# CameronDiao/MolCLR

Hardware: AMD Instinct MI355X
Metric: contrastive pre-train molecules/sec at batch 512, 1/2/4/8 MI355X; HBM GB/s on scatter_add (higher is better)
Workload: dtype f32; 1 GPU; c2: GIN 5x300 feat 512, batch 512/GPU, 10-50 atom graphs; model=gin 5x300 feat 512, global_batch=512, per_gpu_batch=512, mean_nodes_per_view=15278, mean_edges_per_view=25094, parallelism=dp1, views=one paired encoder pass, per-view BatchNorm statistics, augment=host: pre-built resident batch pairs

## Files before the change

### include/molclr.h

```cpp
#ifndef MOLCLR_H_
#define MOLCLR_H_

#include <stddef.h>
#include <stdint.h>

#ifdef __cplusplus
extern "C" {
#endif

typedef void* molclr_stream_t;

enum {
  MOLCLR_OK = 0,
  MOLCLR_ERR_ARG = -1,
  MOLCLR_ERR_WORKSPACE = -2,
  MOLCLR_ERR_UNSUPPORTED = -3
};

#define MOLCLR_NUM_ATOM_TYPE 119
#define MOLCLR_NUM_CHIRALITY 3
#define MOLCLR_NUM_BOND_TYPE 5
#define MOLCLR_NUM_BOND_DIR 3
#define MOLCLR_SELF_LOOP_BOND_TYPE 4
#define MOLCLR_ECOUNT_STRIDE 8
// ... 32 lines not shown
                             molclr_stream_t stream);

typedef struct molclr_stage_source {
  const int64_t *x, *edge_index, *edge_attr, *batch;
  int64_t num_nodes, num_edges;
} molclr_stage_source;
typedef struct molclr_graph_staged_segment {
  const int64_t* edge_index;
  const int64_t* edge_attr;
  const int64_t* batch;
  int64_t node_cap, edge_cap, num_graphs;
} molclr_graph_staged_segment;
int molclr_stage_segments(int nseg, const molclr_stage_source* src,
                          const molclr_graph_staged_segment* dst, int64_t* x_all,
                          int64_t num_nodes_cap, int64_t num_edges_cap, int64_t* counts,
                          molclr_stream_t stream);
int molclr_graph_build_dev(int nseg, const molclr_graph_staged_segment* segs, const int64_t* counts,
                           int64_t num_nodes_cap, int64_t num_edges_cap, int32_t* rowptr,
                           int32_t* col, uint8_t* ecode, int32_t* rowptr_t, int32_t* col_t,
                           uint32_t* nbr, uint32_t* nbr_t, int32_t* ecount, int32_t* graph_ptr,
                           int32_t* status, void* workspace, size_t workspace_bytes,
                           molclr_stream_t stream);

size_t molclr_mask_views_workspace_bytes(int64_t batch_size);
int molclr_mask_views(const int64_t* store_x, const int64_t* store_atom_ptr,
                      const int64_t* store_edge_index, const int64_t* store_edge_attr,
                      const int64_t* store_bond_ptr, int64_t store_mols, int64_t store_edges,
                      const int64_t* mol_ids, int64_t batch_size, uint64_t seed, int view,
                      int64_t* x_out, int64_t* edge_index_out, int64_t* edge_attr_out,
                      int64_t* batch_out, int64_t* ptr_out, int64_t num_nodes, int64_t num_edges,
                      int32_t* status, void* workspace, size_t workspace_bytes,
                      molclr_stream_t stream);

enum { MOLCLR_AUG_SUBGRAPH = 0, MOLCLR_AUG_MIX = 1 };
size_t molclr_aug_views_workspace_bytes(int64_t batch_size, int64_t num_nodes, int64_t num_bonds);
int molclr_aug_views_plan(const int64_t* store_atom_ptr, const int64_t* store_edge_index,
                          const int64_t* store_bond_ptr, int64_t store_mols, int64_t store_edges,
                          const int64_t* mol_ids, int64_t batch_size, uint64_t seed, int view,
                          int mode, int64_t num_nodes, int64_t num_bonds, int64_t* ptr_out,
                          int64_t* num_edges_out, int32_t* status, void* workspace,
                          size_t workspace_bytes, molclr_stream_t stream);
size_t molclr_aug_views_big_workspace_bytes(int64_t big_slots, int64_t big_atoms,
                                            int64_t big_bonds);
int molclr_aug_views_plan_big(const int64_t* store_atom_ptr, const int64_t* store_edge_index,
                              const int64_t* store_bond_ptr, int64_t store_mols,
                              int64_t store_edges, const int64_t* mol_ids, int64_t batch_size,
                              uint64_t seed, int view, int mode, int64_t num_nodes,
                              int64_t num_bonds, int64_t* ptr_out, int64_t* num_edges_out,
                              int32_t* status, void* workspace, size_t workspace_bytes,
                              int64_t big_slots, int64_t big_atoms, int64_t big_bonds,
                              void* big_workspace, size_t big_workspace_bytes,
                              molclr_stream_t stream);
int molclr_aug_views_write(const int64_t* store_x, const int64_t* store_atom_ptr,
                           const int64_t* store_edge_index, const int64_t* store_edge_attr,
                           const int64_t* store_bond_ptr, int64_t store_mols, int64_t store_edges,
                           const int64_t* mol_ids, int64_t batch_size, const int64_t* ptr,
                           int64_t num_nodes, int64_t num_bonds, int64_t num_edges, int64_t* x_out,
                           int64_t* edge_index_out, int64_t* edge_attr_out, int64_t* batch_out,
                           const void* workspace, size_t workspace_bytes, molclr_stream_t stream);

int molclr_atom_embed_fwd(const int64_t* x, const float* X1, const float* X2,
                          float* h, int64_t num_nodes, int64_t dim, int64_t n1,
                          int64_t n2, int32_t* status, molclr_stream_t stream);
size_t molclr_atom_embed_bwd_workspace_bytes(int64_t num_nodes, int64_t dim, int64_t n1,
                                             int64_t n2);
int molclr_atom_embed_bwd(const int64_t* x, const float* dh, float* dX1, float* dX2,
                          int64_t num_nodes, int64_t dim, int64_t n1, int64_t n2, int accumulate,
                          void* workspace, size_t workspace_bytes, molclr_stream_t stream);

#define MOLCLR_MAX_LAYERS 16
int molclr_edge_tables_combine(int layers, const float* const* E1s, const float* const* E2s,
                               float* Ec, int64_t dim, molclr_stream_t stream);

int molclr_gine_aggregate_fwd(const float* x, const int32_t* rowptr, const int32_t* col,
                              const uint8_t* ecode, const uint32_t* nbr, const float* Ec,
                              float* out, int64_t num_nodes, int64_t dim,
                              molclr_stream_t stream);
int64_t molclr_rowmax_layout(int64_t D);
size_t molclr_rowmax_bytes(int64_t N, int64_t D);
int molclr_gine_aggregate_fwd_rowmax(const float* x, const int32_t* rowptr, const int32_t* col,
                                     const uint8_t* ecode, const uint32_t* nbr, const float* Ec,
                                     float* out, int64_t N, int64_t D, float* rowparts,
                                     float* slot, molclr_stream_t stream);
size_t molclr_gine_aggregate_bwd_workspace_bytes(int64_t num_nodes, int64_t dim);
int molclr_gine_aggregate_bwd(const float* g, const int32_t* rowptr_t, const int32_t* col_t,
                              const uint32_t* nbr_t, const int32_t* ecount, float* dx, float* dE1, float* dE2,
                              int64_t num_nodes, int64_t dim, int accumulate, void* workspace,
                              size_t workspace_bytes, molclr_stream_t stream);

int molclr_gcn_aggregate_fwd(const float* xw, const int32_t* rowptr, const int32_t* col,
                             const uint8_t* ecode, const uint32_t* nbr, const float* E1,
                             const float* E2,
                             const float* bias, float* out, int64_t num_nodes,
                             int64_t dim, molclr_stream_t stream);
size_t molclr_gcn_aggregate_bwd_workspace_bytes(int64_t num_nodes, int64_t dim);
int molclr_gcn_aggregate_bwd(const float* g, const int32_t* rowptr_t, const int32_t* col_t,
                             const uint32_t* nbr_t, const int32_t* ecount, float* dxw, float* dE1, float* dE2,
                             float* dbias, int64_t num_nodes, int64_t dim, int accumulate,
                             void* workspace, size_t workspace_bytes, molclr_stream_t stream);

enum { MOLCLR_EPI_NONE = 0, MOLCLR_EPI_BIAS = 1, MOLCLR_EPI_BIAS_RELU = 2,
       MOLCLR_EPI_RELU_MASK = 3,
       MOLCLR_EPI_ACCUMULATE = 16  };
size_t molclr_gemm_f32_workspace_bytes(int64_t M, int64_t N, int64_t K);
int molclr_gemm_f32(const float* A, const float* B, float* C, int64_t M, int64_t N,
                    int64_t K, int64_t lda, int64_t ldb, int64_t ldc, int a_kmajor,
                    int b_kmajor, int epilogue_flags, const float* bias, const float* aux,
                    int64_t ldaux, void* workspace, size_t workspace_bytes,
                    molclr_stream_t stream);

int molclr_gemm_f32_impl(const float* A, const float* B, float* C, int64_t M, int64_t N,
                         int64_t K, int64_t lda, int64_t ldb, int64_t ldc, int a_kmajor,
                         int b_kmajor, int epilogue_flags, const float* bias, const float* aux,
                         int64_t ldaux, void* workspace, size_t workspace_bytes,
                         molclr_stream_t stream, int impl);

size_t molclr_bplanes_bytes(int64_t N, int64_t K);
int molclr_bplanes_make(const float* B, int64_t N, int64_t K, int64_t ldb, int b_kmajor,
                        uint16_t* planes, molclr_stream_t stream);
int molclr_bplanes_make_batch(int count, const float* const* B, const int64_t* N,
                              const int64_t* K, const int64_t* ldb, const int* b_kmajor,
                              uint16_t* const* planes, molclr_stream_t stream);
int molclr_gemm_f32_bplanes(const float* A, const uint16_t* planes, float* C, int64_t M,
                            int64_t N, int64_t K, int64_t lda, int64_t ldc, int a_kmajor,
                            int epilogue_flags, const float* bias, const float* aux,
                            int64_t ldaux, void* workspace, size_t workspace_bytes,
                            molclr_stream_t stream);
int molclr_gemm_f32_bplanes_tile(const float* A, const uint16_t* planes, float* C, int64_t M,
                                 int64_t N, int64_t K, int64_t lda, int64_t ldc, int a_kmajor,
                                 int epilogue_flags, const float* bias, const float* aux,
                                 int64_t ldaux, void* workspace, size_t workspace_bytes,
                                 molclr_stream_t stream, int tile);

size_t molclr_linear_wgrad_workspace_bytes(int64_t rows, int64_t n_out, int64_t n_in);
int molclr_linear_wgrad(const float* dy, const float* x, float* dW, float* db, int64_t rows,
                        int64_t n_out, int64_t n_in, int64_t ld_dy, int64_t ld_x, int accumulate,
                        void* workspace, size_t workspace_bytes, molclr_stream_t stream);
int molclr_linear_wgrad_groups(const float* dy, const float* x, float* dW, float* db,
                               int64_t rows, int64_t n_out, int64_t n_in, int64_t ld_dy,
                               int64_t ld_x, int accumulate, void* workspace,
                               size_t workspace_bytes, molclr_stream_t stream, int groups);

int molclr_absmax_f32(const float* x, int64_t rows, int64_t cols, int64_t ld, float* slot,
                      int accumulate, molclr_stream_t stream);
size_t molclr_hplanes_bytes(int64_t N, int64_t K);
int molclr_hplanes_make_batch(int count, const float* const* B, const int64_t* N,
                              const int64_t* K, const int64_t* ldb, const int* b_kmajor,
                              uint16_t* const* planes, molclr_stream_t stream);
int64_t molclr_gemm_row_parts(int64_t N);
int molclr_gemm_f32_bplanes_max(const float* A, const uint16_t* planes, float* C, int64_t M,
                                int64_t N, int64_t K, int64_t lda, int64_t ldc,
                                int epilogue_flags, const float* bias, const float* aux,
                                int64_t ldaux, float* amax_out, float* cmax, float* crow,
                                uint32_t* relu_bits, void* workspace, size_t workspace_bytes,
                                molclr_stream_t stream);
int molclr_absmax_rows_f32(const float* x, int64_t rows, int64_t cols, int64_t ld,
                           float* rowmax, float* slot, int accumulate, molclr_stream_t stream);
int molclr_gemm_f32_h3(const float* A, const float* amax, int a_row_parts, const uint16_t* hplanes,
                       float* C, int64_t M, int64_t N, int64_t K, int64_t lda, int64_t ldc,
                       int epilogue_flags, const float* bias, const float* aux, int64_t ldaux,
                       const uint32_t* mask_bits, float* cmax, float* crow, float* amax_out,
                       molclr_stream_t stream);
int molclr_gemm_f32_h3_impl(const float* A, const float* amax, int a_row_parts,
                            const uint16_t* hplanes, float* C, int64_t M, int64_t N, int64_t K,
                            int64_t lda, int64_t ldc, int epilogue_flags, const float* bias,
                            const float* aux, int64_t ldaux, const uint32_t* mask_bits, float* cmax,
                            float* crow, float* amax_out, uint32_t* relu_bits,
                            molclr_stream_t stream, int impl);
int molclr_gemm_f32_h3_bits(const float* A, const float* amax, int a_row_parts,
                            const uint16_t* hplanes, float* C, int64_t M, int64_t N, int64_t K,
                            int64_t lda, int64_t ldc, int epilogue_flags, const float* bias,
                            const float* aux, int64_t ldaux, const uint32_t* mask_bits,
                            float* cmax, float* crow, float* amax_out, uint32_t* relu_bits,
                            molclr_stream_t stream);
int molclr_linear_wgrad_h3_groups(const float* dy, const float* dymax, const float* x,
                                  const float* xmax, float* dW, float* db, int64_t rows,
                                  int64_t n_out, int64_t n_in, int64_t ld_dy, int64_t ld_x,
                                  int accumulate, void* workspace, size_t workspace_bytes,
                                  molclr_stream_t stream, int groups);
int molclr_linear_wgrad_h3(const float* dy, const float* dymax, const float* x,
                           const float* xmax, float* dW, float* db, int64_t rows, int64_t n_out,
                           int64_t n_in, int64_t ld_dy, int64_t ld_x, int accumulate,
                           void* workspace, size_t workspace_bytes, molclr_stream_t stream);
size_t molclr_linear_wgrad_h3_pair_workspace_bytes(int64_t rows, int64_t n_out_a, int64_t n_in_a,
                                                   int64_t n_out_b, int64_t n_in_b);
int molclr_linear_wgrad_h3_pair(const float* dy_a, const float* dymax_a, const float* x_a,
                                const float* xmax_a, float* dW_a, float* db_a, int64_t n_out_a,
                                int64_t n_in_a, int64_t ld_dy_a, int64_t ld_x_a,
                                const float* dy_b, const float* dymax_b, const float* x_b,
                                const float* xmax_b, float* dW_b, float* db_b, int64_t n_out_b,
                                int64_t n_in_b, int64_t ld_dy_b, int64_t ld_x_b, int64_t rows,
                                int accumulate, void* workspace, size_t workspace_bytes,
                                molclr_stream_t stream);

size_t molclr_colsum_f32_workspace_bytes(int64_t rows, int64_t cols);
int molclr_colsum_f32(const float* X, float* out, int64_t rows, int64_t cols, int64_t ld,
                      int accumulate, void* workspace, size_t workspace_bytes,
                      molclr_stream_t stream);

size_t molclr_batchnorm_workspace_bytes(int64_t rows, int64_t dim);
int molclr_batchnorm_fwd(const float* z, const float* gamma, const float* beta,
                         float* running_mean, float* running_var,
                         int64_t* num_batches_tracked, float* y,
                         float* save_mean, float* save_invstd, int64_t rows, int64_t dim,
                         double momentum, double eps, int training, int relu,
                         void* workspace, size_t workspace_bytes, molclr_stream_t stream);
int molclr_batchnorm_bwd(const float* dy, const float* z, const float* gamma,
                         const float* beta, const float* save_mean,
                         const float* save_invstd, float* dz, float* dgamma, float* dbeta,
                         int64_t rows, int64_t dim, int relu, int accumulate, void* workspace,
                         size_t workspace_bytes, molclr_stream_t stream);

enum { MOLCLR_DTYPE_F32 = 0, MOLCLR_DTYPE_BF16 = 1 };
size_t molclr_batchnorm_seg_workspace_bytes(int nseg, const int64_t* seg_rows, int64_t dim);
int molclr_batchnorm_seg_fwd(const void* z, const float* gamma, const float* beta,
                             float* running_mean, float* running_var,
                             int64_t* num_batches_tracked, void* y, float* save_mean,
                             float* save_invstd, int nseg, const int64_t* seg_rows, int64_t dim,
                             int dtype, double momentum, double eps, int training, int relu,
                             void* workspace, size_t workspace_bytes, molclr_stream_t stream);
int molclr_batchnorm_seg_bwd(const void* dy, const void* z, const float* gamma,
                             const float* beta, const float* save_mean, const float* save_invstd,
                             void* dz, float* dgamma, float* dbeta, int nseg,
                             const int64_t* seg_rows, int64_t dim, int dtype, int relu,
                             int accumulate, void* workspace, size_t workspace_bytes,
                             molclr_stream_t stream);

int molclr_bn_row_parts(int64_t dim);
size_t molclr_batchnorm_seg_dev_workspace_bytes(int nseg, int64_t rows_cap, int64_t dim);
int molclr_batchnorm_seg_fwd_dev(const void* z, const float* gamma, const float* beta,
                                 float* running_mean, float* running_var,
                                 int64_t* num_batches_tracked, void* y, float* save_mean,
                                 float* save_invstd, int nseg, const int64_t* seg_rows_dev,
                                 int64_t rows_cap, int64_t dim, int dtype, double momentum,
                                 double eps, int training, int relu, void* workspace,
                                 size_t workspace_bytes, molclr_stream_t stream);
int molclr_batchnorm_seg_bwd_dev(const void* dy, const void* z, const float* gamma,
                                 const float* beta, const float* save_mean,
                                 const float* save_invstd, void* dz, float* dgamma, float* dbeta,
                                 int nseg, const int64_t* seg_rows_dev, int64_t rows_cap,
                                 int64_t dim, int dtype, int relu, int accumulate, float* rowmax,
                                 float* slot, void* workspace, size_t workspace_bytes,
                                 molclr_stream_t stream);
int molclr_batchnorm_seg_bwd_max(const float* dy, const float* z, const float* gamma,
                                 const float* beta, const float* save_mean,
                                 const float* save_invstd, float* dz, float* dgamma, float* dbeta,
                                 int nseg, const int64_t* seg_rows, int64_t dim, int relu,
                                 int accumulate, float* rowmax, float* slot, void* workspace,
                                 size_t workspace_bytes, molclr_stream_t stream);

int molclr_segment_pool_fwd(const float* h, const int32_t* graph_ptr, float* out,
                            int64_t num_graphs, int64_t dim, int mode,
                            molclr_stream_t stream);
int molclr_segment_pool_bwd(const float* dout, const int32_t* graph_ptr, float* dh,
                            int64_t num_nodes, int64_t num_graphs, int64_t dim, int mode,
                            molclr_stream_t stream);
int molclr_segment_max_fwd(const void* h, const int32_t* graph_ptr, float* out, int32_t* argmax,
                           int64_t num_graphs, int64_t dim, int dtype, molclr_stream_t stream);
int molclr_segment_max_bwd(const float* dout, const int32_t* argmax, void* dh, int64_t num_nodes,
                           int64_t num_graphs, int64_t dim, int dtype, molclr_stream_t stream);

int molclr_l2norm_fwd(const float* z, float* y, float* norm, int64_t rows, int64_t dim,
                      double eps, molclr_stream_t stream);
int molclr_l2norm_bwd(const float* dy, const float* y, const float* norm, float* dz,
                      int64_t rows, int64_t dim, double eps, molclr_stream_t stream);

int molclr_ntxent_prep(const float* r, float* rhat, float* norm, int64_t n, int64_t C,
                       int cosine, molclr_stream_t stream);
int molclr_ntxent_prep_bwd(const float* drhat, const float* rhat, const float* norm,
                           float* dr, int64_t n, int64_t C, int cosine,
                           molclr_stream_t stream);
int molclr_ntxent_prep_pair(const float* z, float* y, float* rhat, float* n1, float* n2,
                            int64_t batch_local, int64_t C, double eps, int cosine,
                            molclr_stream_t stream);
int molclr_ntxent_prep_pair_bwd(const float* drhat, const float* rhat, const float* n2,
                                const float* y, const float* n1, float* dz, int64_t batch_local,
                                int64_t C, double eps, int cosine, molclr_stream_t stream);
size_t molclr_ntxent_workspace_bytes(int64_t nrows, int64_t ncols, int64_t C);
int molclr_ntxent_fwd(const float* rhat_rows, const int32_t* row_gidx, const float* rhat_cols,
                      int64_t nrows, int64_t ncols, int64_t C, int64_t batch_size,
                      double temperature, float* lse_rows, float* loss_rows,
                      void* workspace, size_t workspace_bytes, molclr_stream_t stream);
int molclr_ntxent_bwd(const float* rhat_rows, const int32_t* row_gidx, const float* rhat_cols,
                      const float* lse_cols, const float* grad_loss, int64_t nrows,
                      int64_t ncols, int64_t C, int64_t batch_size, double temperature,
                      float* drhat_rows, void* workspace, size_t workspace_bytes,
                      molclr_stream_t stream);
size_t molclr_ntxent_sim_bytes(int64_t nrows, int64_t ncols, int64_t C, int impl);
int molclr_ntxent_fwd_impl(const float* rhat_rows, const int32_t* row_gidx,
                           const float* rhat_cols, int64_t nrows, int64_t ncols, int64_t C,
                           int64_t batch_size, double temperature, float* lse_rows,
                           float* loss_rows, float* sim, void* workspace, size_t workspace_bytes,
                           molclr_stream_t stream, int impl);
int molclr_ntxent_bwd_impl(const float* rhat_rows, const int32_t* row_gidx,
                           const float* rhat_cols, const float* lse_cols, const float* grad_loss,
                           int64_t nrows, int64_t ncols, int64_t C, int64_t batch_size,
                           double temperature, const float* sim, float* drhat_rows,
                           void* workspace, size_t workspace_bytes, molclr_stream_t stream,
                           int impl);
int molclr_sum_f32(const float* x, float* out, int64_t n, molclr_stream_t stream);

int molclr_adam_step(float* param, const float* grad, float* exp_avg, float* exp_avg_sq,
                     int64_t n, const float* lr, int32_t* step, double beta1, double beta2,
                     double eps, double weight_decay, molclr_stream_t stream);
int molclr_adam_step_ex(float* param, const float* grad, float* exp_avg, float* exp_avg_sq,
                        int64_t n, const float* lr, int32_t* step, double beta1, double beta2,
                        double eps, double weight_decay, int tick, molclr_stream_t stream);
int molclr_step_tail(int32_t* step, const float* loss_src, float* loss_dst,
                     const int32_t* status_src, int32_t* status_acc, molclr_stream_t stream);

typedef struct molclr_gin_encoder {
  int32_t num_layer;
  int32_t training;
  int64_t dim;
  int64_t n_atom;
  int64_t n_chiral;
  double momentum, eps;
  const float* x_embedding1;
  const float* x_embedding2;
// ... 33 lines not shown
} molclr_gin_encoder_grads;

typedef struct molclr_device_graph {
  int64_t num_nodes, num_edges, num_graphs;
  const int32_t *rowptr, *col, *rowptr_t, *col_t, *ecount, *graph_ptr;
  const uint8_t* ecode;
  const uint32_t *nbr, *nbr_t;
  int32_t num_segments;
  int64_t segment_nodes[MOLCLR_MAX_SEGMENTS];
  const int64_t* segment_nodes_dev;
} molclr_device_graph;

size_t molclr_gin_encoder_arena_bytes(int num_layer, int64_t num_nodes, int64_t dim, int dtype);
size_t molclr_gin_encoder_workspace_bytes(int num_layer, int64_t num_nodes, int64_t dim,
                                          int dtype);
int molclr_gin_encoder_fwd(const molclr_gin_encoder* enc, const int64_t* x,
                           const molclr_device_graph* graph, void* h_out, void* arena,
                           size_t arena_bytes, void* workspace, size_t workspace_bytes,
                           molclr_stream_t stream);
int molclr_gin_encoder_bwd(const molclr_gin_encoder* enc, const molclr_gin_encoder_grads* grads,
                           const int64_t* x, const molclr_device_graph* graph,
                           const void* dh_out, const void* arena, size_t arena_bytes,
                           void* workspace, size_t workspace_bytes, molclr_stream_t stream);

typedef struct molclr_gcn_encoder {
  int32_t num_layer;
  int32_t training;
  int64_t dim;
  int64_t n_atom;
  int64_t n_chiral;
  double momentum, eps;
  const float* x_embedding1;
  const float* x_embedding2;
  const float* weight[MOLCLR_MAX_LAYERS];
  const float* bias[MOLCLR_MAX_LAYERS];
  const float* edge_embedding1[MOLCLR_MAX_LAYERS];
  const float* edge_embedding2[MOLCLR_MAX_LAYERS];
  const float* bn_weight[MOLCLR_MAX_LAYERS];
  const float* bn_bias[MOLCLR_MAX_LAYERS];
  float* bn_running_mean[MOLCLR_MAX_LAYERS];
  float* bn_running_var[MOLCLR_MAX_LAYERS];
  int64_t* bn_num_batches_tracked[MOLCLR_MAX_LAYERS];
  const uint16_t* weight_planes[MOLCLR_MAX_LAYERS];
  const uint16_t* weight_planes_t[MOLCLR_MAX_LAYERS];
  int32_t fp32_gemm;
  int32_t* status;
} molclr_gcn_encoder;

typedef struct molclr_gcn_encoder_grads {
  float* x_embedding1;
  float* x_embedding2;
  float* weight[MOLCLR_MAX_LAYERS];
  float* bias[MOLCLR_MAX_LAYERS];
  float* edge_embedding1[MOLCLR_MAX_LAYERS];
  float* edge_embedding2[MOLCLR_MAX_LAYERS];
  float* bn_weight[MOLCLR_MAX_LAYERS];
  float* bn_bias[MOLCLR_MAX_LAYERS];
  void* layer_done[MOLCLR_MAX_LAYERS];
  void* embed_done;
} molclr_gcn_encoder_grads;

size_t molclr_gcn_encoder_arena_bytes(int num_layer, int64_t num_nodes, int64_t dim);
size_t molclr_gcn_encoder_workspace_bytes(int num_layer, int64_t num_nodes, int64_t dim);
int molclr_gcn_encoder_fwd(const molclr_gcn_encoder* enc, const int64_t* x,
                           const molclr_device_graph* graph, float* h_out, void* arena,
                           size_t arena_bytes, void* workspace, size_t workspace_bytes,
                           molclr_stream_t stream);
int molclr_gcn_encoder_bwd(const molclr_gcn_encoder* enc, const molclr_gcn_encoder_grads* grads,
                           const int64_t* x, const molclr_device_graph* graph,
                           const float* dh_out, const void* arena, size_t arena_bytes,
                           void* workspace, size_t workspace_bytes, molclr_stream_t stream);

int molclr_atom_embed_fwd_bf16(const int64_t* x, const float* X1, const float* X2, uint16_t* h,
                               int64_t num_nodes, int64_t dim, int64_t n1, int64_t n2,
                               int32_t* status, molclr_stream_t stream);
int molclr_atom_embed_bwd_bf16(const int64_t* x, const uint16_t* dh, float* dX1, float* dX2,
                               int64_t num_nodes, int64_t dim, int64_t n1, int64_t n2,
                               int accumulate, void* workspace, size_t workspace_bytes,
                               molclr_stream_t stream);
int molclr_gine_aggregate_fwd_bf16(const uint16_t* x, const int32_t* rowptr, const int32_t* col,
                                   const uint8_t* ecode, const uint32_t* nbr, const float* Ec,
                                   uint16_t* out, int64_t num_nodes, int64_t dim,
                                   molclr_stream_t stream);
int molclr_gine_aggregate_bwd_bf16(const uint16_t* g, const int32_t* rowptr_t,
                                   const int32_t* col_t, const uint32_t* nbr_t,
                                   const int32_t* ecount, uint16_t* dx, float* dE1, float* dE2,
                                   int64_t num_nodes, int64_t dim, int accumulate, void* workspace,
                                   size_t workspace_bytes, molclr_stream_t stream);
int molclr_segment_pool_fwd_bf16(const uint16_t* h, const int32_t* graph_ptr, float* out,
                                 int64_t num_graphs, int64_t dim, int mode,
                                 molclr_stream_t stream);
int molclr_segment_pool_bwd_bf16(const float* dout, const int32_t* graph_ptr, uint16_t* dh,
                                 int64_t num_nodes, int64_t num_graphs, int64_t dim, int mode,
                                 molclr_stream_t stream);
int molclr_gemm_bf16(const uint16_t* A, const uint16_t* planes, uint16_t* C, int64_t M, int64_t N,
                     int64_t K, int64_t lda, int64_t ldc, int epilogue, const float* bias,
                     const uint16_t* aux, int64_t ldaux, molclr_stream_t stream);
int molclr_gemm_bf16_impl(const uint16_t* A, const uint16_t* planes, uint16_t* C, int64_t M,
                          int64_t N, int64_t K, int64_t lda, int64_t ldc, int epilogue,
                          const float* bias, const uint16_t* aux, int64_t ldaux,
                          molclr_stream_t stream, int impl);
int molclr_gemm_bf16_bits(const uint16_t* A, const uint16_t* planes, uint16_t* C, int64_t M,
                          int64_t N, int64_t K, int64_t lda, int64_t ldc, int epilogue,
                          const float* bias, uint32_t* bits_out, const uint32_t* bits_in,
                          molclr_stream_t stream);
size_t molclr_linear_wgrad_bf16_workspace_bytes(int64_t rows, int64_t n_out, int64_t n_in);
int molclr_linear_wgrad_bf16(const uint16_t* dy, const uint16_t* x, float* dW, float* db,
                             int64_t rows, int64_t n_out, int64_t n_in, int64_t ld_dy,
                             int64_t ld_x, int accumulate, void* workspace,
                             size_t workspace_bytes, molclr_stream_t stream);
int molclr_linear_wgrad_bf16_impl(const uint16_t* dy, const uint16_t* x, float* dW, float* db,
                                  int64_t rows, int64_t n_out, int64_t n_in, int64_t ld_dy,
                                  int64_t ld_x, int accumulate, void* workspace,
                                  size_t workspace_bytes, molclr_stream_t stream, int impl);

#define MOLCLR_KTIMER_GINE_AGG 1
#define MOLCLR_KTIMER_GEMM 2
#define MOLCLR_KTIMER_NTXENT 4
#define MOLCLR_KTIMER_GCN_AGG 8
int molclr_ktimer_start(int kinds_mask);
int molclr_ktimer_read(int kind, double* total_ms, int64_t* launches);
int molclr_ktimer_stop(void);

#ifdef __cplusplus
}
#endif
#endif
```

### molclr_amd/_lib.py

```python
from __future__ import annotations

import ctypes
import os
from ctypes import POINTER, c_char_p, c_double, c_int, c_int64, c_size_t, c_uint64, c_void_p
from pathlib import Path

import torch

LIB_PATH = Path(os.environ.get("MOLCLR_LIB", Path(__file__).resolve().parent / "libmolclr_hip.so"))

_P = c_void_p
_I64 = c_int64

SIGNATURES = {
    "molclr_version": (c_char_p, []),
    "molclr_last_error": (c_char_p, []),
    "molclr_graph_build_workspace_bytes": (c_size_t, [_I64, _I64]),
    "molclr_graph_build": (c_int, [_P, _P, _P, _I64, _I64, _I64, _P, _P, _P, _P, _P, _P, _P, _P,
                                   _P, _P, _P, c_size_t, _P]),
    "molclr_graph_build_multi": (c_int, [c_int, _P, _P, _P, _P, _P, _P, _P, _P, _P, _P, _P, _P,
                                         c_size_t, _P]),
    "molclr_stage_segments": (c_int, [c_int, _P, _P, _P, _I64, _I64, _P, _P]),
    "molclr_graph_build_dev": (c_int, [c_int, _P, _P, _I64, _I64, _P, _P, _P, _P, _P, _P, _P, _P,
                                       _P, _P, _P, c_size_t, _P]),
    "molclr_mask_views_workspace_bytes": (c_size_t, [_I64]),
    "molclr_mask_views": (c_int, [_P, _P, _P, _P, _P, _I64, _I64, _P, _I64, c_uint64, c_int, _P, _P,
                                  _P, _P, _P, _I64, _I64, _P, _P, c_size_t, _P]),
    "molclr_atom_embed_fwd": (c_int, [_P, _P, _P, _P, _I64, _I64, _I64, _I64, _P, _P]),
    "molclr_atom_embed_bwd_workspace_bytes": (c_size_t, [_I64, _I64, _I64, _I64]),
    "molclr_atom_embed_bwd": (c_int, [_P, _P, _P, _P, _I64, _I64, _I64, _I64, c_int, _P, c_size_t,
                                      _P]),
    "molclr_edge_tables_combine": (c_int, [c_int, _P, _P, _P, _I64, _P]),
    "molclr_gine_aggregate_fwd": (c_int, [_P, _P, _P, _P, _P, _P, _P, _I64, _I64, _P]),
    "molclr_rowmax_layout": (_I64, [_I64]),
    "molclr_rowmax_bytes": (c_size_t, [_I64, _I64]),
    "molclr_gine_aggregate_fwd_rowmax": (c_int, [_P, _P, _P, _P, _P, _P, _P, _I64, _I64, _P, _P,
                                                 _P]),
    "molclr_gine_aggregate_bwd_workspace_bytes": (c_size_t, [_I64, _I64]),
    "molclr_gine_aggregate_bwd": (c_int, [_P, _P, _P, _P, _P, _P, _P, _P, _I64, _I64, c_int, _P,
                                          c_size_t, _P]),
    "molclr_gcn_aggregate_fwd": (c_int, [_P, _P, _P, _P, _P, _P, _P, _P, _P, _I64, _I64, _P]),
    "molclr_gcn_aggregate_bwd_workspace_bytes": (c_size_t, [_I64, _I64]),
    "molclr_gcn_aggregate_bwd": (c_int, [_P, _P, _P, _P, _P, _P, _P, _P, _P, _I64, _I64, c_int,
                                         _P, c_size_t, _P]),
    "molclr_gemm_f32_workspace_bytes": (c_size_t, [_I64, _I64, _I64]),
    "molclr_gemm_f32": (c_int, [_P, _P, _P, _I64, _I64, _I64, _I64, _I64, _I64, c_int, c_int, c_int,
                                _P, _P, _I64, _P, c_size_t, _P]),
    "molclr_gemm_f32_impl": (c_int, [_P, _P, _P, _I64, _I64, _I64, _I64, _I64, _I64, c_int, c_int,
                                     c_int, _P, _P, _I64, _P, c_size_t, _P, c_int]),
    "molclr_bplanes_bytes": (c_size_t, [_I64, _I64]),
    "molclr_bplanes_make": (c_int, [_P, _I64, _I64, _I64, c_int, _P, _P]),
    "molclr_bplanes_make_batch": (c_int, [c_int, _P, _P, _P, _P, _P, _P, _P]),
    "molclr_gemm_f32_bplanes": (c_int, [_P, _P, _P, _I64, _I64, _I64, _I64, _I64, c_int, c_int, _P,
                                        _P, _I64, _P, c_size_t, _P]),
    "molclr_gemm_f32_bplanes_tile": (c_int, [_P, _P, _P, _I64, _I64, _I64, _I64, _I64, c_int,
                                             c_int, _P, _P, _I64, _P, c_size_t, _P, c_int]),
    "molclr_linear_wgrad_workspace_bytes": (c_size_t, [_I64, _I64, _I64]),
    "molclr_linear_wgrad": (c_int, [_P, _P, _P, _P, _I64, _I64, _I64, _I64, _I64, c_int, _P, c_size_t,
                                    _P]),
    "molclr_linear_wgrad_groups": (c_int, [_P, _P, _P, _P, _I64, _I64, _I64, _I64, _I64, c_int, _P,
                                           c_size_t, _P, c_int]),
    "molclr_absmax_f32": (c_int, [_P, _I64, _I64, _I64, _P, c_int, _P]),
    "molclr_hplanes_bytes": (c_size_t, [_I64, _I64]),
    "molclr_hplanes_make_batch": (c_int, [c_int, _P, _P, _P, _P, _P, _P, _P]),
    "molclr_absmax_rows_f32": (c_int, [_P, _I64, _I64, _I64, _P, _P, c_int, _P]),
    "molclr_bn_row_parts": (c_int, [_I64]),
    "molclr_batchnorm_seg_bwd_max": (c_int, [_P, _P, _P, _P, _P, _P, _P, _P, _P, c_int, _P, _I64,
                                             c_int, c_int, _P, _P, _P, c_size_t, _P]),
    "molclr_gemm_row_parts": (_I64, [_I64]),
    "molclr_gemm_f32_bplanes_max": (c_int, [_P, _P, _P, _I64, _I64, _I64, _I64, _I64, c_int, _P,
                                            _P, _I64, _P, _P, _P, _P, _P, c_size_t, _P]),
    "molclr_gemm_f32_h3": (c_int, [_P, _P, c_int, _P, _P, _I64, _I64, _I64, _I64, _I64, c_int, _P,
                                   _P, _I64, _P, _P, _P, _P, _P]),
    "molclr_gemm_f32_h3_bits": (c_int, [_P, _P, c_int, _P, _P, _I64, _I64, _I64, _I64, _I64, c_int,
                                        _P, _P, _I64, _P, _P, _P, _P, _P, _P]),
    "molclr_gemm_f32_h3_impl": (c_int, [_P, _P, c_int, _P, _P, _I64, _I64, _I64, _I64, _I64, c_int,
                                        _P, _P, _I64, _P, _P, _P, _P, _P, _P, c_int]),
    "molclr_linear_wgrad_h3_groups": (c_int, [_P, _P, _P, _P, _P, _P, _I64, _I64, _I64, _I64, _I64,
                                              c_int, _P, c_size_t, _P, c_int]),
    "molclr_linear_wgrad_h3": (c_int, [_P, _P, _P, _P, _P, _P, _I64, _I64, _I64, _I64, _I64, c_int,
                                       _P, c_size_t, _P]),
    "molclr_colsum_f32_workspace_bytes": (c_size_t, [_I64, _I64]),
    "molclr_colsum_f32": (c_int, [_P, _P, _I64, _I64, _I64, c_int, _P, c_size_t, _P]),
    "molclr_batchnorm_workspace_bytes": (c_size_t, [_I64, _I64]),
    "molclr_batchnorm_fwd": (c_int, [_P, _P, _P, _P, _P, _P, _P, _P, _P, _I64, _I64, c_double,
                                     c_double, c_int, c_int, _P, c_size_t, _P]),
    "molclr_batchnorm_bwd": (c_int, [_P, _P, _P, _P, _P, _P, _P, _P, _P, _I64, _I64, c_int, c_int,
                                     _P, c_size_t, _P]),
    "molclr_batchnorm_seg_workspace_bytes": (c_size_t, [c_int, _P, _I64]),
    "molclr_batchnorm_seg_fwd": (c_int, [_P, _P, _P, _P, _P, _P, _P, _P, _P, c_int, _P, _I64, c_int,
                                         c_double, c_double, c_int, c_int, _P, c_size_t, _P]),
    "molclr_batchnorm_seg_bwd": (c_int, [_P, _P, _P, _P, _P, _P, _P, _P, _P, c_int, _P, _I64, c_int,
                                         c_int, c_int, _P, c_size_t, _P]),
    "molclr_batchnorm_seg_dev_workspace_bytes": (c_size_t, [c_int, _I64, _I64]),
    "molclr_batchnorm_seg_fwd_dev": (c_int, [_P, _P, _P, _P, _P, _P, _P, _P, _P, c_int, _P, _I64,
                                             _I64, c_int, c_double, c_double, c_int, c_int, _P,
                                             c_size_t, _P]),
    "molclr_batchnorm_seg_bwd_dev": (c_int, [_P, _P, _P, _P, _P, _P, _P, _P, _P, c_int, _P, _I64,
                                             _I64, c_int, c_int, c_int, _P, _P, _P, c_size_t, _P]),
    "molclr_segment_pool_fwd": (c_int, [_P, _P, _P, _I64, _I64, c_int, _P]),
    "molclr_segment_pool_bwd": (c_int, [_P, _P, _P, _I64, _I64, _I64, c_int, _P]),
    "molclr_l2norm_fwd": (c_int, [_P, _P, _P, _I64, _I64, c_double, _P]),
    "molclr_l2norm_bwd": (c_int, [_P, _P, _P, _P, _I64, _I64, c_double, _P]),
    "molclr_ntxent_prep": (c_int, [_P, _P, _P, _I64, _I64, c_int, _P]),
    "molclr_ntxent_prep_bwd": (c_int, [_P, _P, _P, _P, _I64, _I64, c_int, _P]),
    "molclr_ntxent_prep_pair": (c_int, [_P, _P, _P, _P, _P, _I64, _I64, c_double, c_int, _P]),
    "molclr_ntxent_prep_pair_bwd": (c_int, [_P, _P, _P, _P, _P, _P, _I64, _I64, c_double, c_int,
                                            _P]),
    "molclr_ntxent_workspace_bytes": (c_size_t, [_I64, _I64, _I64]),
    "molclr_ntxent_fwd": (c_int, [_P, _P, _P, _I64, _I64, _I64, _I64, c_double, _P, _P, _P,
                                  c_size_t, _P]),
    "molclr_ntxent_bwd": (c_int, [_P, _P, _P, _P, _P, _I64, _I64, _I64, _I64, c_double, _P, _P,
                                  c_size_t, _P]),
    "molclr_ntxent_sim_bytes": (c_size_t, [_I64, _I64, _I64, c_int]),
    "molclr_ntxent_fwd_impl": (c_int, [_P, _P, _P, _I64, _I64, _I64, _I64, c_double, _P, _P,
                                       _P, _P, c_size_t, _P, c_int]),
    "molclr_ntxent_bwd_impl": (c_int, [_P, _P, _P, _P, _P, _I64, _I64, _I64, _I64, c_double, _P,
                                       _P, _P, c_size_t, _P, c_int]),
    "molclr_sum_f32": (c_int, [_P, _P, _I64, _P]),
    "molclr_linear_wgrad_h3_pair_workspace_bytes": (c_size_t, [_I64, _I64, _I64, _I64, _I64]),
# ... 185 lines not shown
```

### molclr_amd/csrc/aggregate.hip

```cpp
#include "common.h"

#include <stdlib.h>

namespace {

constexpr int kT = 256;

template <typename St, int U = 1>
__global__ void k_atom_embed_fwd(const int64_t* __restrict__ x, const float4* __restrict__ X1,
                                 const float4* __restrict__ X2, typename St::T* __restrict__ h,
                                 int64_t N, int d4, int64_t n1, int64_t n2,
                                 int32_t* __restrict__ status) {
  int64_t t = (int64_t)blockIdx.x * blockDim.x + threadIdx.x;
  if (t >= N * d4 / U) return;
  const int64_t u0 = t * U;
  int64_t i = N * d4 < (1ll << 32) ? (int64_t)((uint32_t)u0 / (uint32_t)d4) : u0 / d4;
  int c = (int)(u0 - i * d4);
  const int64_t a = x[2 * i], b = x[2 * i + 1];
  float4 v[U];
  if (a < 0 || a >= n1 || b < 0 || b >= n2) {
    const float q = __builtin_nanf("");
#pragma unroll
    for (int j = 0; j < U; ++j) v[j] = make_float4(q, q, q, q);
    if (c == 0 && status != nullptr) atomicOr(status, MOLCLR_STATUS_ATOM_RANGE);
// ... 160 lines not shown
  const int64_t col = (int64_t)blockIdx.y * 64 + lane;
  double acc = 0.0;
  if (col < D) {
    int32_t ch = kchunk0[k] + w;
    const int32_t ce = kchunk0[k + 1];
    for (; ch + 7 * kEmbFinW < ce; ch += 8 * kEmbFinW) {
      double v[8];
#pragma unroll
      for (int u = 0; u < 8; ++u) v[u] = csum[(int64_t)(ch + u * kEmbFinW) * D + col];
#pragma unroll
      for (int u = 0; u < 8; ++u) acc += v[u];
    }
    for (; ch < ce; ch += kEmbFinW) acc += csum[(int64_t)ch * D + col];
  }
  red[w][lane] = acc;
  __syncthreads();
  if (w != 0 || col >= D) return;
  double t = red[0][lane];
#pragma unroll
  for (int q = 1; q < kEmbFinW; ++q) t += red[q][lane];
  float* o = k < n1 ? dX1 + k * D + col : dX2 + (k - n1) * D + col;
  *o = accumulate ? *o + (float)t : (float)t;
}

__global__ __launch_bounds__(1024) void k_reduce_partials_split(
    const double* __restrict__ partial, int64_t P, int64_t rows, int64_t D, int64_t split,
    float* __restrict__ outA, float* __restrict__ outB, int accumulate) {
  constexpr int EL = 16, LANES = 64;
  __shared__ double red[LANES][EL];
  const int cl = threadIdx.x % EL, rl = threadIdx.x / EL;
  const int64_t t = (int64_t)blockIdx.x * EL + cl;
  const int64_t n = rows * D;
  double a0 = 0.0, a1 = 0.0, a2 = 0.0, a3 = 0.0;
  if (t < n) {
    int64_t p = rl;
    for (; p + 3 * LANES < P; p += 4 * LANES) {
      a0 += partial[p * n + t];
      a1 += partial[(p + LANES) * n + t];
      a2 += partial[(p + 2 * LANES) * n + t];
      a3 += partial[(p + 3 * LANES) * n + t];
    }
    for (; p < P; p += LANES) a0 += partial[p * n + t];
  }
  double acc = (a0 + a1) + (a2 + a3);
  red[rl][cl] = acc;
  __syncthreads();
#pragma unroll
  for (int stride = LANES / 2; stride > 0; stride >>= 1) {
    if (rl < stride) red[rl][cl] = acc = acc + red[rl + stride][cl];
    __syncthreads();
  }
  if (rl != 0 || t >= n) return;
  int64_t r = t / D;
  float* o = r < split ? (outA ? outA + t : nullptr) : (outB ? outB + (t - split * D) : nullptr);
  if (o) *o = accumulate ? *o + (float)acc : (float)acc;
}

struct TablePtrs {
  const float* e1[MOLCLR_MAX_LAYERS];
  const float* e2[MOLCLR_MAX_LAYERS];
};
__global__ void k_edge_tables_combine(TablePtrs p, float* __restrict__ Ec, int layers, int64_t D,
                                      float* __restrict__ zero, int64_t n_zero) {
  const int64_t per = (int64_t)MOLCLR_NUM_ECOMB * D;
  int64_t t = (int64_t)blockIdx.x * blockDim.x + threadIdx.x;
  if (t < n_zero) zero[t] = 0.f;
  if (t >= layers * per) return;
  const int l = (int)(t / per);
  const int64_t rc = t - l * per;
  const int r = (int)(rc / D);
  const int64_t c = rc - (int64_t)r * D;
  Ec[t] = p.e1[l][(r / 3) * D + c] + p.e2[l][(r % 3) * D + c];
}

__device__ __forceinline__ uint32_t nbr_degree(uint32_t w0) { return w0 >> 29; }
__device__ __forceinline__ int32_t nbr_node(uint32_t w) { return (int32_t)(w & 0xFFFFFFu); }
__device__ __forceinline__ int nbr_ecomb(uint32_t w) { return (int)((w >> 24) & 15u); }

__device__ __forceinline__ float4 gine_msg(const float4* __restrict__ x, const float4* __restrict__ Ec,
                                           uint32_t w, int d4, int c) {
  return f4add(x[(int64_t)nbr_node(w) * d4 + c], Ec[nbr_ecomb(w) * d4 + c]);
}

template <typename St, bool NT = false>
__device__ __forceinline__ float4 gine_agg_elem(
    const typename St::T* __restrict__ x, const int32_t* __restrict__ rowptr,
    const int32_t* __restrict__ col, const uint8_t* __restrict__ ecode,
    const uint4* __restrict__ nbr, const float4* __restrict__ Ec, typename St::T* __restrict__ out,
    int64_t t, int64_t i, int c, int d4) {
  auto X = [&](int64_t idx) { return St::ld(x, idx); };
  auto msg = [&](uint32_t w) {
    return f4add(X((int64_t)nbr_node(w) * d4 + c), Ec[nbr_ecomb(w) * d4 + c]);
  };
  const uint4 s = nbr[i];
  const float4 self = X(t);
  const float4 es = Ec[MOLCLR_SELF_LOOP_ECOMB * d4 + c];
  const uint32_t deg = nbr_degree(s.x);
  float4 acc = f4zero();
  if (deg <= MOLCLR_NBR_SLOTS) {
    const float4 m0 = deg > 0 ? msg(s.x) : acc;
    const float4 m1 = deg > 1 ? msg(s.y) : acc;
    const float4 m2 = deg > 2 ? msg(s.z) : acc;
    const float4 m3 = deg > 3 ? msg(s.w) : acc;
    if (deg > 0) acc = f4add(acc, m0);
    if (deg > 1) acc = f4add(acc, m1);
    if (deg > 2) acc = f4add(acc, m2);
    if (deg > 3) acc = f4add(acc, m3);
  } else {
    for (int32_t k = rowptr[i], e = rowptr[i + 1]; k < e; ++k)
      acc = f4add(acc, f4add(X((int64_t)col[k] * d4 + c), Ec[MOLCLR_ECOMB(ecode[k]) * d4 + c]));
  }
  acc = f4add(acc, f4add(self, es));
  if constexpr (NT) {
    typedef float f4v __attribute__((ext_vector_type(4)));
    __builtin_nontemporal_store(f4v{acc.x, acc.y, acc.z, acc.w}, reinterpret_cast<f4v*>(out) + t);
  } else {
    St::st(out, t, acc);
  }
  return acc;
}

template <typename St, bool ROWMAX, bool NT = false>
__global__ __launch_bounds__(kT) void k_gine_agg_fwd(
    const typename St::T* __restrict__ x, const int32_t* __restrict__ rowptr,
    const int32_t* __restrict__ col, const uint8_t* __restrict__ ecode,
    const uint4* __restrict__ nbr, const float4* __restrict__ Ec, typename St::T* __restrict__ out,
    int64_t N, int d4, float* __restrict__ rowparts, int nparts, float* __restrict__ slot) {
  int64_t t = (int64_t)xcd_remap(blockIdx.x, gridDim.x) * blockDim.x + threadIdx.x;
  int64_t i;
  int c;
  if (N * d4 < (1ll << 32)) {
    const uint32_t q = (uint32_t)t / (uint32_t)d4;
    i = q;
    c = (int)((uint32_t)t - q * (uint32_t)d4);
  } else {
    i = t / d4;
    c = (int)(t - i * d4);
  }
  if constexpr (ROWMAX) {
    float m = 0.f;
    int row = -1;
    if (t < N * d4) {
      const float4 v = gine_agg_elem<St, NT>(x, rowptr, col, ecode, nbr, Ec, out, t, i, c, d4);
      m = fmaxf(fmaxf(fabsf(v.x), fabsf(v.y)), fmaxf(fabsf(v.z), fabsf(v.w)));
      row = (int)i;
    }
    if (nparts < 0)
      row_max_waves(m, row, t, N, d4, reinterpret_cast<float2*>(rowparts));
    else
      row_max_parts(m, row, t, N, d4, rowparts, nparts);
    if (slot != nullptr) absmax_publish(m, slot);
    return;
  }
  if (t >= N * d4) return;
  gine_agg_elem<St, NT>(x, rowptr, col, ecode, nbr, Ec, out, t, i, c, d4);
}

template <typename St = StF32>
__global__ __launch_bounds__(kT) void k_transpose_gather(const typename St::T* __restrict__ g,
                                                         const int32_t* __restrict__ rowptr_t,
                                                         const int32_t* __restrict__ col_t,
                                                         const uint4* __restrict__ nbr_t,
                                                         typename St::T* __restrict__ dx, int64_t N,
                                                         int d4) {
  int64_t t = (int64_t)xcd_remap(blockIdx.x, gridDim.x) * blockDim.x + threadIdx.x;
  if (t >= N * d4) return;
  int64_t j = N * d4 < (1ll << 32) ? (int64_t)((uint32_t)t / (uint32_t)d4) : t / d4;
  int c = (int)(t - j * d4);
  const uint4 s = nbr_t[j];
  const uint32_t deg = nbr_degree(s.x);
  float4 acc = f4zero();
  if (deg <= MOLCLR_NBR_SLOTS) {
    if (deg > 0) acc = f4add(acc, St::ld(g, (int64_t)nbr_node(s.x) * d4 + c));
    if (deg > 1) acc = f4add(acc, St::ld(g, (int64_t)nbr_node(s.y) * d4 + c));
    if (deg > 2) acc = f4add(acc, St::ld(g, (int64_t)nbr_node(s.z) * d4 + c));
    if (deg > 3) acc = f4add(acc, St::ld(g, (int64_t)nbr_node(s.w) * d4 + c));
  } else {
    for (int32_t k = rowptr_t[j], e = rowptr_t[j + 1]; k < e; ++k)
      acc = f4add(acc, St::ld(g, (int64_t)col_t[k] * d4 + c));
  }
  St::st(dx, t, f4add(acc, St::ld(g, t)));
}

template <typename St = StF32>
__global__ void k_ecount_weighted_partial(const typename St::T* __restrict__ g,
                                          const int32_t* __restrict__ ecount, int64_t N, int d4,
                                          int band, int64_t rows_per_part,
                                          double* __restrict__ partial) {
  extern __shared__ __attribute__((aligned(16))) float4 red[];
  const int tid = threadIdx.x;
  const bool live = tid < band * d4;
  const int r = live ? tid / d4 : 0, c = live ? tid - r * d4 : 0;
  const int64_t beg = (int64_t)blockIdx.x * rows_per_part;
  int64_t end = beg + rows_per_part;
  if (end > N) end = N;
  float4 acc[8];
#pragma unroll
  for (int s = 0; s < 8; ++s) acc[s] = f4zero();
  if (live) {
    constexpr int U = 8;
    for (int64_t i0 = beg + r; i0 < end; i0 += U * (int64_t)band) {
      int4 lo[U], hi[U];
      float4 v[U];
#pragma unroll
      for (int u = 0; u < U; ++u) {
        const int64_t i = i0 + (int64_t)u * band;
        const bool in = i < end;
        const int4* ec = reinterpret_cast<const int4*>(ecount + (in ? i : beg) * 8);
        lo[u] = ec[0];
        hi[u] = ec[1];
        v[u] = St::ld(g, (in ? i : beg) * d4 + c);
      }
#pragma unroll
      for (int u = 0; u < U; ++u) {
        if (i0 + (int64_t)u * band >= end) break;
        const int cnt[8] = {lo[u].x, lo[u].y, lo[u].z, lo[u].w, hi[u].x, hi[u].y, hi[u].z, hi[u].w};
#pragma unroll
        for (int s = 0; s < 8; ++s) {
          const float w = (float)cnt[s];
          acc[s].x += w * v[u].x;
          acc[s].y += w * v[u].y;
          acc[s].z += w * v[u].z;
          acc[s].w += w * v[u].w;
        }
      }
    }
#pragma unroll
    for (int s = 0; s < 8; ++s) red[(r * 8 + s) * d4 + c] = acc[s];
  }
  __syncthreads();
  if (!live || r != 0) return;
  double* out = partial + (int64_t)blockIdx.x * 8 * (4 * d4);
#pragma unroll
  for (int s = 0; s < 8; ++s) {
    double x = 0.0, y = 0.0, z = 0.0, w = 0.0;
    for (int q = 0; q < band; ++q) {
      const float4 v = red[(q * 8 + s) * d4 + c];
      x += v.x;
// ... 55 lines not shown
  const int lane = threadIdx.x & 63;
  const int64_t wave = ((int64_t)blockIdx.x * blockDim.x + threadIdx.x) >> 6;
  const int64_t nwaves = ((int64_t)gridDim.x * blockDim.x) >> 6;
  double acc[8] = {0.0, 0.0, 0.0, 0.0, 0.0, 0.0, 0.0, 0.0};
  for (int64_t i = wave; i < N; i += 2 * nwaves) {
    const int64_t i2 = i + nwaves;
    double s = 0.0, s2 = 0.0;
    for (int c = lane; c < d4; c += 64) {
      const float4 v = g[i * d4 + c];
      const float4 v2 = i2 < N ? g[i2 * d4 + c] : f4zero();
      s += ((double)v.x + (double)v.y) + ((double)v.z + (double)v.w);
      s2 += ((double)v2.x + (double)v2.y) + ((double)v2.z + (double)v2.w);
    }
#pragma unroll
    for (int o = 32; o > 0; o >>= 1) {
      s += __shfl_xor(s, o, 64);
      s2 += __shfl_xor(s2, o, 64);
    }
#pragma unroll
    for (int q = 0; q < 8; ++q) acc[q] += (double)ecount[i * 8 + q] * s;
    if (i2 < N) {
#pragma unroll
      for (int q = 0; q < 8; ++q) acc[q] += (double)ecount[i2 * 8 + q] * s2;
    }
  }
  if (lane < 8) {
    double v = acc[0];
#pragma unroll
    for (int q = 1; q < 8; ++q)
      if (lane == q) v = acc[q];
    partial[wave * 8 + lane] = v;
  }
}

__global__ __launch_bounds__(512) void k_reduce_rowsum_partial(
    const double* __restrict__ partial, int64_t nparts, float* __restrict__ dE1,
    float* __restrict__ dE2, int accumulate) {
  constexpr int G = 64;
  __shared__ double red[G][8];
  const int q = threadIdx.x & 7, r = threadIdx.x >> 3;
  double a0 = 0.0, a1 = 0.0, a2 = 0.0, a3 = 0.0;
  int64_t p = r;
  for (; p + 3 * G < nparts; p += 4 * G) {
    a0 += partial[p * 8 + q];
    a1 += partial[(p + G) * 8 + q];
    a2 += partial[(p + 2 * G) * 8 + q];
    a3 += partial[(p + 3 * G) * 8 + q];
  }
  for (; p < nparts; p += G) a0 += partial[p * 8 + q];
  double acc = (a0 + a1) + (a2 + a3);
  red[r][q] = acc;
  __syncthreads();
#pragma unroll
  for (int stride = G / 2; stride > 0; stride >>= 1) {
    if (r < stride) red[r][q] = acc = acc + red[r + stride][q];
    __syncthreads();
  }
  if (r != 0) return;
  float* o = q < 5 ? (dE1 ? dE1 + q : nullptr) : (dE2 ? dE2 + (q - 5) : nullptr);
  if (o) *o = accumulate ? *o + (float)acc : (float)acc;
}

struct F8 {
  float4 a, b;
};
__device__ __forceinline__ F8 ld8(const uint16_t* __restrict__ p, int64_t unit) {
  const uint4 u = reinterpret_cast<const uint4*>(p)[unit];
  return {make_float4(bf16_to_f32(u.x & 0xFFFFu), bf16_to_f32(u.x >> 16), bf16_to_f32(u.y & 0xFFFFu),
                      bf16_to_f32(u.y >> 16)),
          make_float4(bf16_to_f32(u.z & 0xFFFFu), bf16_to_f32(u.z >> 16), bf16_to_f32(u.w & 0xFFFFu),
                      bf16_to_f32(u.w >> 16))};
}
__device__ __forceinline__ void st8(uint16_t* __restrict__ p, int64_t unit, F8 v) {
  reinterpret_cast<uint4*>(p)[unit] =
      make_uint4(f32x2_to_bf16x2(v.a.x, v.a.y), f32x2_to_bf16x2(v.a.z, v.a.w),
                 f32x2_to_bf16x2(v.b.x, v.b.y), f32x2_to_bf16x2(v.b.z, v.b.w));
}
__device__ __forceinline__ F8 f8add(F8 x, F8 y) { return {f4add(x.a, y.a), f4add(x.b, y.b)}; }
__device__ __forceinline__ F8 ec8(const float4* __restrict__ Ec, int comb, int d8, int c) {
  const float4* e = Ec + (int64_t)comb * 2 * d8 + 2 * c;
  return {e[0], e[1]};
}

__global__ __launch_bounds__(kT) void k_gine_agg_fwd_b8(
    const uint16_t* __restrict__ x, const int32_t* __restrict__ rowptr,
    const int32_t* __restrict__ col, const uint8_t* __restrict__ ecode,
    const uint4* __restrict__ nbr, const float4* __restrict__ Ec, uint16_t* __restrict__ out,
    int64_t N, int d8) {
  int64_t t = (int64_t)xcd_remap(blockIdx.x, gridDim.x) * blockDim.x + threadIdx.x;
  if (t >= N * d8) return;
  const int64_t i = t / d8;
  const int c = (int)(t - i * d8);
  auto msg = [&](uint32_t w) {
    return f8add(ld8(x, (int64_t)nbr_node(w) * d8 + c), ec8(Ec, nbr_ecomb(w), d8, c));
  };
  const uint4 s = nbr[i];
  const F8 self = ld8(x, t);
  const F8 es = ec8(Ec, MOLCLR_SELF_LOOP_ECOMB, d8, c);
  const uint32_t deg = nbr_degree(s.x);
  F8 acc = {f4zero(), f4zero()};
  if (deg <= MOLCLR_NBR_SLOTS) {
    const F8 m0 = deg > 0 ? msg(s.x) : acc;
    const F8 m1 = deg > 1 ? msg(s.y) : acc;
    const F8 m2 = deg > 2 ? msg(s.z) : acc;
    const F8 m3 = deg > 3 ? msg(s.w) : acc;
    if (deg > 0) acc = f8add(acc, m0);
    if (deg > 1) acc = f8add(acc, m1);
    if (deg > 2) acc = f8add(acc, m2);
    if (deg > 3) acc = f8add(acc, m3);
  } else {
    for (int32_t k = rowptr[i], e = rowptr[i + 1]; k < e; ++k)
      acc = f8add(acc, f8add(ld8(x, (int64_t)col[k] * d8 + c), ec8(Ec, MOLCLR_ECOMB(ecode[k]), d8, c)));
  }
  st8(out, t, f8add(acc, f8add(self, es)));
}

__global__ __launch_bounds__(kT) void k_transpose_gather_b8(const uint16_t* __restrict__ g,
                                                            const int32_t* __restrict__ rowptr_t,
                                                            const int32_t* __restrict__ col_t,
                                                            const uint4* __restrict__ nbr_t,
                                                            uint16_t* __restrict__ dx, int64_t N,
                                                            int d8) {
  int64_t t = (int64_t)xcd_remap(blockIdx.x, gridDim.x) * blockDim.x + threadIdx.x;
  if (t >= N * d8) return;
  const int64_t j = t / d8;
  const int c = (int)(t - j * d8);
  const uint4 s = nbr_t[j];
  const uint32_t deg = nbr_degree(s.x);
  F8 acc = {f4zero(), f4zero()};
  if (deg <= MOLCLR_NBR_SLOTS) {
    if (deg > 0) acc = f8add(acc, ld8(g, (int64_t)nbr_node(s.x) * d8 + c));
    if (deg > 1) acc = f8add(acc, ld8(g, (int64_t)nbr_node(s.y) * d8 + c));
    if (deg > 2) acc = f8add(acc, ld8(g, (int64_t)nbr_node(s.z) * d8 + c));
    if (deg > 3) acc = f8add(acc, ld8(g, (int64_t)nbr_node(s.w) * d8 + c));
  } else {
    for (int32_t k = rowptr_t[j], e = rowptr_t[j + 1]; k < e; ++k)
      acc = f8add(acc, ld8(g, (int64_t)col_t[k] * d8 + c));
  }
  st8(dx, t, f8add(acc, ld8(g, t)));
}

int64_t ecount_parts(int64_t N, int band) {
  int64_t P = molclr::ceil_div(N, (int64_t)band * 8);
  if (P > 1024) P = 1024;
  if (P < 1) P = 1;
  return P;
}
constexpr int64_t kRowsumBlocks = 1024;

}

int molclr_colsum_impl(const float* X, float* out, int64_t rows, int64_t cols, int64_t ld,
                       int accumulate, molclr::Workspace& w, hipStream_t s);
size_t molclr_colsum_ws(int64_t rows, int64_t cols);

MOLCLR_API int molclr_atom_embed_fwd(const int64_t* x, const float* X1, const float* X2,
                                     float* h, int64_t N, int64_t D, int64_t n1, int64_t n2,
                                     int32_t* status, molclr_stream_t stream) {
  MOLCLR_REQUIRE(D > 0 && D % 4 == 0, "atom_embed_fwd: dim %lld must be a positive multiple of 4",
                 (long long)D);
  MOLCLR_REQUIRE(n1 > 0 && n2 > 0, "atom_embed_fwd: empty table");
  if (N == 0) return MOLCLR_OK;
  MOLCLR_REQUIRE(x && X1 && X2 && h, "atom_embed_fwd: null pointer");
  int d4 = (int)(D / 4);
  hipLaunchKernelGGL(k_atom_embed_fwd<StF32>, dim3(molclr::ceil_div(N * d4, kT)), dim3(kT), 0,
                     molclr::as_stream(stream), x, (const float4*)X1, (const float4*)X2, h, N, d4,
                     n1, n2, status);
  MOLCLR_LAUNCHED();
  return MOLCLR_OK;
}

namespace {
struct EmbWs {
  int32_t *hist, *total, *kstart, *cbeg, *cend, *kchunk0, *nchunks, *perm;
  double* csum;
  int64_t nblk, max_chunks;
};
EmbWs emb_ws(void* w, size_t bytes, int64_t N, int64_t D, int64_t n1, int64_t n2) {
  molclr::Workspace ws(w, bytes);
  EmbWs e;
  const int64_t nk = n1 + n2;
  e.nblk = molclr::ceil_div(2 * N > 0 ? 2 * N : 1, (int64_t)kEmbBlock);
  e.max_chunks = molclr::ceil_div(2 * N, (int64_t)kEmbChunk) + nk;
  e.hist = ws.take<int32_t>(e.nblk * nk);
  e.total = ws.take<int32_t>(nk);
  e.kstart = ws.take<int32_t>(nk + 1);
  e.kchunk0 = ws.take<int32_t>(nk + 1);
  e.cbeg = ws.take<int32_t>(e.max_chunks);
  e.cend = ws.take<int32_t>(e.max_chunks);
  e.nchunks = ws.take<int32_t>(1);
  e.perm = ws.take<int32_t>(2 * N > 0 ? 2 * N : 1);
  e.csum = ws.take<double>(e.max_chunks * D);
  return e;
}

// ... 24 lines not shown
                       static_cast<const int32_t*>(e.cbeg), static_cast<const int32_t*>(e.cend),
                       static_cast<const int32_t*>(e.nchunks), d4, e.csum);
  }
  hipLaunchKernelGGL(k_emb_finish, dim3((unsigned)nk, (unsigned)molclr::ceil_div(D, 64)),
                     dim3(64 * kEmbFinW), 0, s,
                     static_cast<const double*>(e.csum), static_cast<const int32_t*>(e.kchunk0), n1,
                     n2, D, dX1, dX2, accumulate);
  MOLCLR_LAUNCHED();
  return MOLCLR_OK;
}
}

MOLCLR_API size_t molclr_atom_embed_bwd_workspace_bytes(int64_t N, int64_t D, int64_t n1,
                                                        int64_t n2) {
  const int64_t nk = n1 + n2;
  const int64_t nblk = molclr::ceil_div(2 * N > 0 ? 2 * N : 1, (int64_t)kEmbBlock);
  const int64_t max_chunks = molclr::ceil_div(2 * N, (int64_t)kEmbChunk) + nk;
  return (size_t)(nblk * nk + nk + 2 * (nk + 1) + 2 * max_chunks + 1 + 2 * N) * sizeof(int32_t) +
         (size_t)max_chunks * D * sizeof(double) + 10 * 256;
}

MOLCLR_API int molclr_atom_embed_bwd(const int64_t* x, const float* dh, float* dX1, float* dX2,
                                     int64_t N, int64_t D, int64_t n1, int64_t n2, int accumulate,
                                     void* workspace, size_t workspace_bytes,
                                     molclr_stream_t stream) {
  MOLCLR_REQUIRE(D > 0 && D % 4 == 0 && n1 > 0 && n2 > 0 && N >= 0,
                 "atom_embed_bwd: bad sizes (dim a multiple of 4)");
  MOLCLR_REQUIRE(n1 + n2 <= 1024, "atom_embed_bwd: tables too large");
  MOLCLR_REQUIRE(2 * N < (1ll << 31), "atom_embed_bwd: too many nodes");
  MOLCLR_REQUIRE_WS(workspace_bytes, molclr_atom_embed_bwd_workspace_bytes(N, D, n1, n2));
  return emb_bwd<StF32>(x, dh, dX1, dX2, N, D, n1, n2, accumulate, workspace, workspace_bytes,
                        molclr::as_stream(stream));
}

MOLCLR_API int molclr_edge_tables_combine(int layers, const float* const* E1s,
                                          const float* const* E2s, float* Ec, int64_t D,
                                          molclr_stream_t stream) {
  return molclr::edge_tables_combine_zero(layers, E1s, E2s, Ec, D, nullptr, 0, stream);
}

int molclr::edge_tables_combine_zero(int layers, const float* const* E1s, const float* const* E2s,
                                     float* Ec, int64_t D, float* zero, int64_t n_zero,
                                     molclr_stream_t stream) {
  MOLCLR_REQUIRE(layers >= 0 && layers <= MOLCLR_MAX_LAYERS && D > 0,
                 "edge_tables_combine: %d layers (max %d), dim %lld", layers, MOLCLR_MAX_LAYERS,
                 (long long)D);
  if (layers == 0) return MOLCLR_OK;
  MOLCLR_REQUIRE(E1s && E2s && Ec, "edge_tables_combine: null pointer");
  TablePtrs p{};
  for (int l = 0; l < layers; ++l) {
    MOLCLR_REQUIRE(E1s[l] && E2s[l], "edge_tables_combine: null table of layer %d", l);
    p.e1[l] = E1s[l];
    p.e2[l] = E2s[l];
  }
  const int64_t n = (int64_t)layers * MOLCLR_NUM_ECOMB * D;
  const int64_t work = n > n_zero ? n : n_zero;
  hipLaunchKernelGGL(k_edge_tables_combine, dim3(molclr::ceil_div(work, kT)), dim3(kT), 0,
                     molclr::as_stream(stream), p, Ec, layers, D, zero, n_zero);
  MOLCLR_LAUNCHED();
  return MOLCLR_OK;
}

static bool agg_nt() {
  static const bool on = [] {
    const char* e = getenv("MOLCLR_AGG_NT");
    return e != nullptr && e[0] == '1';
  }();
  return on;
}

MOLCLR_API int molclr_gine_aggregate_fwd(const float* x, const int32_t* rowptr,
                                         const int32_t* col, const uint8_t* ecode,
                                         const uint32_t* nbr, const float* Ec, float* out,
                                         int64_t N, int64_t D, molclr_stream_t stream) {
  MOLCLR_REQUIRE(D > 0 && D % 4 == 0, "gine_aggregate_fwd: dim %lld must be a multiple of 4",
                 (long long)D);
  if (N == 0) return MOLCLR_OK;
  MOLCLR_REQUIRE(x && rowptr && nbr && Ec && out, "gine_aggregate_fwd: null pointer");
  int d4 = (int)(D / 4);
  molclr::launch_timed(molclr::kTimeGineAgg, agg_nt() ? k_gine_agg_fwd<StF32, false, true>
                                                      : k_gine_agg_fwd<StF32, false, false>,
                       dim3(molclr::ceil_div(N * d4, kT)), dim3(kT), 0, molclr::as_stream(stream),
                       x, rowptr, col, ecode, (const uint4*)nbr, (const float4*)Ec, out, N, d4,
                       nullptr, 0, nullptr);
  MOLCLR_LAUNCHED();
  return MOLCLR_OK;
}

MOLCLR_API int64_t molclr_rowmax_layout(int64_t D) {
  const int64_t d4 = D / 4;
  return d4 >= 64 ? -d4 : (int64_t)molclr_bn_row_parts(D);
}
MOLCLR_API size_t molclr_rowmax_bytes(int64_t N, int64_t D) {
  const int64_t code = molclr_rowmax_layout(D);
  return code < 0 ? (size_t)((N * (D / 4) + 63) / 64) * 2 * sizeof(float)
                  : (size_t)code * N * sizeof(float);
}

MOLCLR_API int molclr_gine_aggregate_fwd_rowmax(const float* x, const int32_t* rowptr,
                                                const int32_t* col, const uint8_t* ecode,
                                                const uint32_t* nbr, const float* Ec, float* out,
                                                int64_t N, int64_t D, float* rowparts, float* slot,
                                                molclr_stream_t stream) {
  MOLCLR_REQUIRE(D > 0 && D % 4 == 0, "gine_aggregate_fwd_rowmax: dim %lld must be a multiple of 4",
                 (long long)D);
  MOLCLR_REQUIRE(N < (1ll << 31), "gine_aggregate_fwd_rowmax: too many rows");
  if (N == 0) return MOLCLR_OK;
  MOLCLR_REQUIRE(x && rowptr && nbr && Ec && out && rowparts,
                 "gine_aggregate_fwd_rowmax: null pointer");
  const int d4 = (int)(D / 4);
  static_assert(kT % 64 == 0, "row parts follow the waves");
  molclr::launch_timed(molclr::kTimeGineAgg, agg_nt() ? k_gine_agg_fwd<StF32, true, true>
                                                      : k_gine_agg_fwd<StF32, true, false>,
                       dim3(molclr::ceil_div(N * d4, kT)), dim3(kT), 0, molclr::as_stream(stream),
                       x, rowptr, col, ecode, (const uint4*)nbr, (const float4*)Ec, out, N, d4,
                       rowparts, (int)molclr_rowmax_layout(D), slot);
  MOLCLR_LAUNCHED();
  return MOLCLR_OK;
}

MOLCLR_API size_t molclr_gine_aggregate_bwd_workspace_bytes(int64_t N, int64_t D) {
  return (size_t)ecount_parts(N, molclr::make_band(D).band) * 8 * D * sizeof(double) + 256;
}

MOLCLR_API int molclr_gine_aggregate_bwd(const float* g, const int32_t* rowptr_t,
                                         const int32_t* col_t, const uint32_t* nbr_t,
                                         const int32_t* ecount, float* dx,
                                         float* dE1, float* dE2, int64_t N, int64_t D,
                                         int accumulate, void* workspace, size_t workspace_bytes,
                                         molclr_stream_t stream) {
  MOLCLR_REQUIRE(D > 0 && D % 4 == 0, "gine_aggregate_bwd: dim must be a multiple of 4");
  hipStream_t s = molclr::as_stream(stream);
  int d4 = (int)(D / 4);
  if (dx && N > 0) {
    MOLCLR_REQUIRE(g && rowptr_t && nbr_t, "gine_aggregate_bwd: null pointer");
    hipLaunchKernelGGL(k_transpose_gather<StF32>, dim3(molclr::ceil_div(N * d4, kT)), dim3(kT), 0,
                       s, g, rowptr_t, col_t, (const uint4*)nbr_t, dx, N, d4);
  }
  if (dE1 || dE2) {
    MOLCLR_REQUIRE_WS(workspace_bytes, molclr_gine_aggregate_bwd_workspace_bytes(N, D));
    molclr::Band b = molclr::make_band(D);
    int64_t P = ecount_parts(N, b.band);
    int64_t rpp = molclr::ceil_div(N > 0 ? N : 1, P);
    double* partial = (double*)workspace;
    size_t lds = (size_t)b.band * 8 * b.d4 * sizeof(float4);
    MOLCLR_REQUIRE(lds <= 65536, "gine_aggregate_bwd: dim too large for the edge-table reduction");
    hipLaunchKernelGGL(k_ecount_weighted_partial<StF32>, dim3(P), dim3(b.threads), lds, s, g,
                       ecount, N, d4, b.band, rpp, partial);
    hipLaunchKernelGGL(k_reduce_partials_split, dim3(molclr::ceil_div(8 * D, 16)), dim3(1024), 0, s,
                       partial, P, (int64_t)8, D, (int64_t)5, dE1, dE2, accumulate);
  }
  MOLCLR_LAUNCHED();
  return MOLCLR_OK;
}

MOLCLR_API int molclr_gcn_aggregate_fwd(const float* xw, const int32_t* rowptr,
                                        const int32_t* col, const uint8_t* ecode,
                                        const uint32_t* nbr, const float* E1, const float* E2,
                                        const float* bias,
                                        float* out, int64_t N, int64_t D,
                                        molclr_stream_t stream) {
  MOLCLR_REQUIRE(D > 0 && D % 4 == 0, "gcn_aggregate_fwd: dim must be a multiple of 4");
  if (N == 0) return MOLCLR_OK;
  MOLCLR_REQUIRE(xw && rowptr && nbr && E1 && E2 && bias && out, "gcn_aggregate_fwd: null pointer");
  int d4 = (int)(D / 4);
  molclr::launch_timed(molclr::kTimeGcnAgg, k_gcn_agg_fwd,
                       dim3(molclr::ceil_div(N * d4, kT)), dim3(kT), 0, molclr::as_stream(stream),
                       (const float4*)xw, rowptr, col, ecode, (const uint4*)nbr, E1, E2,
                       (const float4*)bias, (float4*)out, N, d4);
  MOLCLR_LAUNCHED();
  return MOLCLR_OK;
}

MOLCLR_API size_t molclr_gcn_aggregate_bwd_workspace_bytes(int64_t N, int64_t D) {
  size_t a = (size_t)kRowsumBlocks * 4 * 8 * sizeof(double) + 256;
  return a + molclr_colsum_ws(N, D);
}

MOLCLR_API int molclr_gcn_aggregate_bwd(const float* g, const int32_t* rowptr_t,
                                        const int32_t* col_t, const uint32_t* nbr_t,
                                        const int32_t* ecount, float* dxw,
                                        float* dE1, float* dE2, float* dbias, int64_t N,
                                        int64_t D, int accumulate, void* workspace,
                                        size_t workspace_bytes, molclr_stream_t stream) {
  MOLCLR_REQUIRE(D > 0 && D % 4 == 0, "gcn_aggregate_bwd: dim must be a multiple of 4");
  MOLCLR_REQUIRE_WS(workspace_bytes, molclr_gcn_aggregate_bwd_workspace_bytes(N, D));
  hipStream_t s = molclr::as_stream(stream);
  int d4 = (int)(D / 4);
  if (dxw && N > 0) {
    MOLCLR_REQUIRE(g && rowptr_t && nbr_t, "gcn_aggregate_bwd: null pointer");
    hipLaunchKernelGGL(k_transpose_gather<StF32>, dim3(molclr::ceil_div(N * d4, kT)), dim3(kT), 0,
                       s, g, rowptr_t, col_t, (const uint4*)nbr_t, dxw, N, d4);
  }
  molclr::Workspace w(workspace, workspace_bytes);
  double* partial = w.take<double>(kRowsumBlocks * 4 * 8);
  if (dE1 || dE2) {
    hipLaunchKernelGGL(k_rowsum_ecount_partial, dim3(kRowsumBlocks), dim3(256), 0, s,
                       (const float4*)g, ecount, N, d4, partial);
    hipLaunchKernelGGL(k_reduce_rowsum_partial, dim3(1), dim3(512), 0, s, partial,
                       kRowsumBlocks * 4, dE1, dE2, accumulate);
  }
  MOLCLR_LAUNCHED();
  if (dbias) {
    int rc = molclr_colsum_impl(g, dbias, N, D, D, accumulate, w, s);
    if (rc) return rc;
  }
  return MOLCLR_OK;
}

MOLCLR_API int molclr_atom_embed_fwd_bf16(const int64_t* x, const float* X1, const float* X2,
                                          uint16_t* h, int64_t N, int64_t D, int64_t n1,
                                          int64_t n2, int32_t* status, molclr_stream_t stream) {
  MOLCLR_REQUIRE(D > 0 && D % 4 == 0, "atom_embed_fwd_bf16: dim must be a multiple of 4");
  MOLCLR_REQUIRE(n1 > 0 && n2 > 0, "atom_embed_fwd_bf16: empty table");
  if (N == 0) return MOLCLR_OK;
  MOLCLR_REQUIRE(x && X1 && X2 && h, "atom_embed_fwd_bf16: null pointer");
  const int d4 = (int)(D / 4);
  if (d4 % 2 == 0)
    hipLaunchKernelGGL((k_atom_embed_fwd<StBF16, 2>), dim3(molclr::ceil_div(N * d4 / 2, kT)),
                       dim3(kT), 0, molclr::as_stream(stream), x, (const float4*)X1,
                       (const float4*)X2, h, N, d4, n1, n2, status);
  else
    hipLaunchKernelGGL((k_atom_embed_fwd<StBF16, 1>), dim3(molclr::ceil_div(N * d4, kT)), dim3(kT),
                       0, molclr::as_stream(stream), x, (const float4*)X1, (const float4*)X2, h, N,
                       d4, n1, n2, status);
  MOLCLR_LAUNCHED();
  return MOLCLR_OK;
}

MOLCLR_API int molclr_atom_embed_bwd_bf16(const int64_t* x, const uint16_t* dh, float* dX1,
                                          float* dX2, int64_t N, int64_t D, int64_t n1, int64_t n2,
                                          int accumulate, void* workspace, size_t workspace_bytes,
                                          molclr_stream_t stream) {
  MOLCLR_REQUIRE(D > 0 && D % 4 == 0 && n1 > 0 && n2 > 0 && N >= 0,
                 "atom_embed_bwd_bf16: bad sizes (dim a multiple of 4)");
  MOLCLR_REQUIRE(n1 + n2 <= 1024, "atom_embed_bwd_bf16: tables too large");
  MOLCLR_REQUIRE(2 * N < (1ll << 31), "atom_embed_bwd_bf16: too many nodes");
  MOLCLR_REQUIRE_WS(workspace_bytes, molclr_atom_embed_bwd_workspace_bytes(N, D, n1, n2));
  return emb_bwd<StBF16>(x, dh, dX1, dX2, N, D, n1, n2, accumulate, workspace, workspace_bytes,
                         molclr::as_stream(stream));
}

MOLCLR_API int molclr_gine_aggregate_fwd_bf16(const uint16_t* x, const int32_t* rowptr,
                                              const int32_t* col, const uint8_t* ecode,
                                              const uint32_t* nbr, const float* Ec, uint16_t* out,
                                              int64_t N, int64_t D, molclr_stream_t stream) {
  MOLCLR_REQUIRE(D > 0 && D % 4 == 0, "gine_aggregate_fwd_bf16: dim must be a multiple of 4");
  if (N == 0) return MOLCLR_OK;
  MOLCLR_REQUIRE(x && rowptr && nbr && Ec && out, "gine_aggregate_fwd_bf16: null pointer");
  if (D % 8 == 0) {
    const int d8 = (int)(D / 8);
    molclr::launch_timed(molclr::kTimeGineAgg, k_gine_agg_fwd_b8, dim3(molclr::ceil_div(N * d8, kT)),
                         dim3(kT), 0, molclr::as_stream(stream), x, rowptr, col, ecode,
                         (const uint4*)nbr, (const float4*)Ec, out, N, d8);
  } else {
    const int d4 = (int)(D / 4);
    molclr::launch_timed(molclr::kTimeGineAgg, k_gine_agg_fwd<StBF16, false>,
                         dim3(molclr::ceil_div(N * d4, kT)), dim3(kT), 0, molclr::as_stream(stream),
                         x, rowptr, col, ecode, (const uint4*)nbr, (const float4*)Ec, out, N, d4,
                         nullptr, 0, nullptr);
  }
  MOLCLR_LAUNCHED();
  return MOLCLR_OK;
}

MOLCLR_API int molclr_gine_aggregate_bwd_bf16(const uint16_t* g, const int32_t* rowptr_t,
                                              const int32_t* col_t, const uint32_t* nbr_t,
                                              const int32_t* ecount, uint16_t* dx, float* dE1,
                                              float* dE2, int64_t N, int64_t D, int accumulate,
                                              void* workspace, size_t workspace_bytes,
                                              molclr_stream_t stream) {
  MOLCLR_REQUIRE(D > 0 && D % 4 == 0, "gine_aggregate_bwd_bf16: dim must be a multiple of 4");
  hipStream_t s = molclr::as_stream(stream);
  const int d4 = (int)(D / 4);
  if (dx && N > 0) {
    MOLCLR_REQUIRE(g && rowptr_t && nbr_t, "gine_aggregate_bwd_bf16: null pointer");
    if (D % 8 == 0)
      hipLaunchKernelGGL(k_transpose_gather_b8, dim3(molclr::ceil_div(N * (D / 8), kT)), dim3(kT), 0,
                         s, g, rowptr_t, col_t, (const uint4*)nbr_t, dx, N, (int)(D / 8));
    else
      hipLaunchKernelGGL(k_transpose_gather<StBF16>, dim3(molclr::ceil_div(N * d4, kT)), dim3(kT),
                         0, s, g, rowptr_t, col_t, (const uint4*)nbr_t, dx, N, d4);
  }
  if (dE1 || dE2) {
    MOLCLR_REQUIRE_WS(workspace_bytes, molclr_gine_aggregate_bwd_workspace_bytes(N, D));
    const molclr::Band b = molclr::make_band(D);
    const int64_t P = ecount_parts(N, b.band);
    const int64_t rpp = molclr::ceil_div(N > 0 ? N : 1, P);
    double* partial = (double*)workspace;
    const size_t lds = (size_t)b.band * 8 * b.d4 * sizeof(float4);
    MOLCLR_REQUIRE(lds <= 65536, "gine_aggregate_bwd_bf16: dim too large for the edge-table reduction");
    hipLaunchKernelGGL(k_ecount_weighted_partial<StBF16>, dim3(P), dim3(b.threads), lds, s, g,
                       ecount, N, d4, b.band, rpp, partial);
    hipLaunchKernelGGL(k_reduce_partials_split, dim3(molclr::ceil_div(8 * D, 16)), dim3(1024), 0, s,
                       partial, P, (int64_t)8, D, (int64_t)5, dE1, dE2, accumulate);
  }
  MOLCLR_LAUNCHED();
  return MOLCLR_OK;
}
```

### molclr_amd/csrc/common.h

```cpp
#pragma once

#include <hip/hip_ext.h>
#include <hip/hip_runtime.h>

#include <type_traits>
#include <stdint.h>
#include <stddef.h>

#include "../../include/molclr.h"

#define MOLCLR_API extern "C" __attribute__((visibility("default")))

namespace molclr {

void set_error(const char* fmt, ...) __attribute__((format(printf, 1, 2)));

inline hipStream_t as_stream(molclr_stream_t s) { return reinterpret_cast<hipStream_t>(s); }

int edge_tables_combine_zero(int layers, const float* const* E1s, const float* const* E2s,
                             float* Ec, int64_t D, float* zero, int64_t n_zero,
                             molclr_stream_t stream);

int hplanes_make_and_max(const float* B, int64_t N, int64_t K, uint16_t* planes, const float* x,
                         int64_t x_rows, int64_t x_cols, float* x_slot, hipStream_t stream);
// ... 155 lines not shown
      return (int)e_;                                                                 \
    }                                                                                 \
  } while (0)

__device__ __forceinline__ float4 f4add(float4 a, float4 b) {
  return make_float4(a.x + b.x, a.y + b.y, a.z + b.z, a.w + b.w);
}
__device__ __forceinline__ int xcd_remap(int bid, int nwg) {
  int q = nwg / 8, r = nwg % 8;
  int x = bid % 8, pos = bid / 8;
  int base = x < r ? x * (q + 1) : r * (q + 1) + (x - r) * q;
  return base + pos;
}

__device__ __forceinline__ float4 f4zero() { return make_float4(0.f, 0.f, 0.f, 0.f); }

__device__ __forceinline__ void wave_lds_sync() {
  __builtin_amdgcn_fence(__ATOMIC_RELEASE, "wavefront");
  __builtin_amdgcn_wave_barrier();
  __builtin_amdgcn_fence(__ATOMIC_ACQUIRE, "wavefront");
}

struct StF32 {
  typedef float T;
  static constexpr int kBytes = 4;
  __device__ __forceinline__ static float4 ld(const T* __restrict__ p, int64_t unit) {
    return reinterpret_cast<const float4*>(p)[unit];
  }
  __device__ __forceinline__ static void st(T* __restrict__ p, int64_t unit, float4 v) {
    reinterpret_cast<float4*>(p)[unit] = v;
  }
  __device__ __forceinline__ static void ld2(const T* __restrict__ p, int64_t u2, float4& a,
                                             float4& b) {
    a = reinterpret_cast<const float4*>(p)[2 * u2];
    b = reinterpret_cast<const float4*>(p)[2 * u2 + 1];
  }
  __device__ __forceinline__ static void st2(T* __restrict__ p, int64_t u2, float4 a, float4 b) {
    reinterpret_cast<float4*>(p)[2 * u2] = a;
    reinterpret_cast<float4*>(p)[2 * u2 + 1] = b;
  }
  __device__ __forceinline__ static float ld1(const T* __restrict__ p, int64_t i) { return p[i]; }
  __device__ __forceinline__ static void st1(T* __restrict__ p, int64_t i, float v) { p[i] = v; }
};

__device__ __forceinline__ float bf16_to_f32(uint32_t bits16) {
  return __uint_as_float(bits16 << 16);
}
__device__ __forceinline__ uint32_t f32x2_to_bf16x2(float a, float b) {
  typedef __bf16 bf2 __attribute__((ext_vector_type(2)));
  const bf2 v = {(__bf16)a, (__bf16)b};
  return __builtin_bit_cast(uint32_t, v);
}

struct StBF16 {
  typedef uint16_t T;
  static constexpr int kBytes = 2;
  __device__ __forceinline__ static float4 ld(const T* __restrict__ p, int64_t unit) {
    const uint2 u = reinterpret_cast<const uint2*>(p)[unit];
    return make_float4(bf16_to_f32(u.x & 0xFFFFu), bf16_to_f32(u.x >> 16),
                       bf16_to_f32(u.y & 0xFFFFu), bf16_to_f32(u.y >> 16));
  }
  __device__ __forceinline__ static void st(T* __restrict__ p, int64_t unit, float4 v) {
    reinterpret_cast<uint2*>(p)[unit] = make_uint2(f32x2_to_bf16x2(v.x, v.y), f32x2_to_bf16x2(v.z, v.w));
  }
  __device__ __forceinline__ static void ld2(const T* __restrict__ p, int64_t u2, float4& a,
                                             float4& b) {
    const uint4 q = reinterpret_cast<const uint4*>(p)[u2];
    a = make_float4(bf16_to_f32(q.x & 0xFFFFu), bf16_to_f32(q.x >> 16), bf16_to_f32(q.y & 0xFFFFu),
                    bf16_to_f32(q.y >> 16));
    b = make_float4(bf16_to_f32(q.z & 0xFFFFu), bf16_to_f32(q.z >> 16), bf16_to_f32(q.w & 0xFFFFu),
                    bf16_to_f32(q.w >> 16));
  }
  __device__ __forceinline__ static void st2(T* __restrict__ p, int64_t u2, float4 a, float4 b) {
    reinterpret_cast<uint4*>(p)[u2] = make_uint4(f32x2_to_bf16x2(a.x, a.y), f32x2_to_bf16x2(a.z, a.w),
                                                 f32x2_to_bf16x2(b.x, b.y), f32x2_to_bf16x2(b.z, b.w));
  }
  __device__ __forceinline__ static float ld1(const T* __restrict__ p, int64_t i) {
    return bf16_to_f32(p[i]);
  }
  __device__ __forceinline__ static void st1(T* __restrict__ p, int64_t i, float v) {
    p[i] = (uint16_t)(f32x2_to_bf16x2(v, 0.f) & 0xFFFFu);
  }
};

__device__ __forceinline__ float wave_sum(float v) {
#pragma unroll
  for (int o = 32; o > 0; o >>= 1) v += __shfl_xor(v, o, 64);
  return v;
}
__device__ __forceinline__ float wave_max_dpp(float v) {
  auto dpp = [](float x, auto ctrl) {
    return __int_as_float(__builtin_amdgcn_update_dpp(0, __float_as_int(x), decltype(ctrl)::value,
                                                      0xF, 0xF, false));
  };
  v = fmaxf(v, dpp(v, std::integral_constant<int, 0xB1>{}));
  v = fmaxf(v, dpp(v, std::integral_constant<int, 0x4E>{}));
  v = fmaxf(v, dpp(v, std::integral_constant<int, 0x141>{}));
  v = fmaxf(v, dpp(v, std::integral_constant<int, 0x140>{}));
  const float a = __int_as_float(__builtin_amdgcn_readlane(__float_as_int(v), 0));
  const float b = __int_as_float(__builtin_amdgcn_readlane(__float_as_int(v), 16));
  const float c = __int_as_float(__builtin_amdgcn_readlane(__float_as_int(v), 32));
  const float d = __int_as_float(__builtin_amdgcn_readlane(__float_as_int(v), 48));
  return fmaxf(fmaxf(a, b), fmaxf(c, d));
}
__device__ __forceinline__ float wave_max(float v) {
#pragma unroll
  for (int o = 32; o > 0; o >>= 1) v = fmaxf(v, __shfl_xor(v, o, 64));
  return v;
}

__device__ __forceinline__ void row_max_parts(float m, int row, int64_t t, int64_t rows, int d4,
                                              float* __restrict__ rowparts, int nparts) {
  const int lane = threadIdx.x & 63;
  if (d4 >= 64) {
    const int64_t t0 = t - lane;
    const int64_t r0 = rows * d4 < (1ll << 32) ? (int64_t)((uint32_t)t0 / (uint32_t)d4) : t0 / d4;
    const bool second = row >= 0 && row != r0;
    const float m0 = wave_max_dpp(second ? 0.f : m), m1 = wave_max_dpp(second ? m : 0.f);
    if (lane == 0 && r0 < rows) {
      const int64_t rs = r0 * d4;
      const int part = (int)((t0 >> 6) - (rs >> 6));
      rowparts[part * rows + r0] = m0;
      if (part == 0)
        for (int q = (int)(((rs + d4 - 1) >> 6) - (rs >> 6)) + 1; q < nparts; ++q)
          rowparts[q * rows + r0] = 0.f;
    }
    const int64_t r1 = r0 + 1, rs1 = r1 * d4;
    if (lane == 1 && r1 < rows && rs1 < t0 + 64) {
      rowparts[r1] = m1;
      for (int q = (int)(((rs1 + d4 - 1) >> 6) - (rs1 >> 6)) + 1; q < nparts; ++q)
        rowparts[q * rows + r1] = 0.f;
    }
    return;
  }
#pragma unroll
  for (int off = 1; off < 64; off <<= 1) {
    const float mv = __shfl_down(m, off, 64);
    const int rv = __shfl_down(row, off, 64);
    if (lane + off < 64 && rv == row) m = fmaxf(m, mv);
  }
  const int rp = __shfl_up(row, 1, 64);
  if (row >= 0 && (lane == 0 || rp != row)) {
    const int64_t rs = (int64_t)row * d4;
    const int part = (int)((t >> 6) - (rs >> 6));
    rowparts[part * rows + row] = m;
    if (part == 0)
      for (int q = (int)(((rs + d4 - 1) >> 6) - (rs >> 6)) + 1; q < nparts; ++q)
        rowparts[q * rows + row] = 0.f;
  }
}

__device__ __forceinline__ void row_max_waves(float m, int row, int64_t t, int64_t rows, int d4,
                                              float2* __restrict__ wm) {
  const int lane = threadIdx.x & 63;
  const int64_t t0 = t - lane;
  const int64_t r0 = rows * d4 < (1ll << 32) ? (int64_t)((uint32_t)t0 / (uint32_t)d4) : t0 / d4;
  const bool second = row >= 0 && row != r0;
  const float m0 = wave_max_dpp(second ? 0.f : m), m1 = wave_max_dpp(second ? m : 0.f);
  if (lane == 0 && t0 < rows * d4) wm[t0 >> 6] = make_float2(m0, m1);
}
__device__ __forceinline__ float row_max_of_waves(const float2* __restrict__ wm, int64_t row,
                                                  int d4) {
  const int64_t s = row * d4, e = s + d4 - 1;
  float m = 0.f;
  for (int64_t w = s >> 6; w <= (e >> 6); ++w) {
    const float2 v = wm[w];
// ... 49 lines not shown
```

### molclr_amd/csrc/encoder.hip

```cpp
#include "common.h"

namespace {

struct ArenaLayout {
  size_t agg[MOLCLR_MAX_LAYERS], a1[MOLCLR_MAX_LAYERS], z[MOLCLR_MAX_LAYERS],
      h[MOLCLR_MAX_LAYERS], mean[MOLCLR_MAX_LAYERS], invstd[MOLCLR_MAX_LAYERS];
  size_t bits[MOLCLR_MAX_LAYERS];
  size_t h0, ec, smax, bmax, total;
  ArenaLayout(int L, int64_t N, int64_t D, size_t es) {
    size_t used = 0;
    auto off = [&](size_t bytes) {
      const size_t o = used;
      used += (bytes + 255) / 256 * 256;
      return o;
    };
    for (int l = 0; l < L; ++l) {
      agg[l] = off(N * D * es);
      a1[l] = off(N * 2 * D * es);
      z[l] = off(N * D * es);
      h[l] = off(N * D * es);
      mean[l] = off(MOLCLR_MAX_SEGMENTS * D * sizeof(float));
      invstd[l] = off(MOLCLR_MAX_SEGMENTS * D * sizeof(float));
      bits[l] = off((size_t)N * ((2 * D + 31) / 32) * sizeof(uint32_t));
    }
    h0 = off(N * D * es);
    ec = off((size_t)L * MOLCLR_NUM_ECOMB * D * sizeof(float));
    smax = off((size_t)MOLCLR_MAX_LAYERS * 2 * kMaxSlotFloats * sizeof(float));
    bmax = off((size_t)MOLCLR_MAX_LAYERS * 2 * kMaxSlotFloats * sizeof(float));
    total = used;
  }
};

size_t elem_bytes(int dtype) { return dtype == MOLCLR_DTYPE_BF16 ? 2 : 4; }

size_t kernels_ws(int64_t N, int64_t D) {
  size_t m = 0;
  auto mx = [&](size_t v) { m = v > m ? v : m; };
  mx(molclr_gemm_f32_workspace_bytes(2 * D, D, N));
  mx(molclr_gemm_f32_workspace_bytes(D, 2 * D, N));
  mx(molclr_gemm_f32_workspace_bytes(N, 2 * D, D));
  mx(molclr_gemm_f32_workspace_bytes(N, D, 2 * D));
  mx(molclr_colsum_f32_workspace_bytes(N, 2 * D));
  mx(molclr_linear_wgrad_workspace_bytes(N, D, 2 * D));
  mx(molclr_linear_wgrad_workspace_bytes(N, 2 * D, D));
  if (N >= 1024 && D % 4 == 0) mx(molclr_linear_wgrad_h3_pair_workspace_bytes(N, D, 2 * D, 2 * D, D));
  mx(molclr_linear_wgrad_bf16_workspace_bytes(N, D, 2 * D));
  mx(molclr_linear_wgrad_bf16_workspace_bytes(N, 2 * D, D));
  mx(molclr_batchnorm_ws_bound(N, D));
  mx(molclr_gine_aggregate_bwd_workspace_bytes(N, D));
  mx(molclr_atom_embed_bwd_workspace_bytes(N, D, MOLCLR_NUM_ATOM_TYPE, MOLCLR_NUM_CHIRALITY));
  return m;
}

size_t scratch_bytes(int64_t N, int64_t D, size_t es) { return ((size_t)N * D * 3 + (size_t)N * 2 * D) * es; }

int check_encoder(const molclr_gin_encoder* e, const molclr_device_graph* g) {
  MOLCLR_REQUIRE(e && g, "gin_encoder: null encoder / graph");
  MOLCLR_REQUIRE(e->num_layer >= 1 && e->num_layer <= MOLCLR_MAX_LAYERS,
                 "gin_encoder: num_layer %d", e->num_layer);
  MOLCLR_REQUIRE(e->dim > 0 && e->dim % 4 == 0, "gin_encoder: dim %lld", (long long)e->dim);
  MOLCLR_REQUIRE(e->dtype == MOLCLR_DTYPE_F32 || (e->dtype == MOLCLR_DTYPE_BF16 && e->dim % 8 == 0),
                 "gin_encoder: dtype %d (bf16 needs dim %% 8 == 0)", e->dtype);
  MOLCLR_REQUIRE(e->n_atom == MOLCLR_NUM_ATOM_TYPE && e->n_chiral == MOLCLR_NUM_CHIRALITY,
                 "gin_encoder: embedding tables must be [%d,D] and [%d,D]",
                 MOLCLR_NUM_ATOM_TYPE, MOLCLR_NUM_CHIRALITY);
  for (int l = 0; l < e->num_layer; ++l)
    MOLCLR_REQUIRE(e->mlp0_planes[l] && e->mlp0_planes_t[l] && e->mlp2_planes[l] &&
                       e->mlp2_planes_t[l] && e->bn_weight[l] && e->bn_bias[l],
                   "gin_encoder: layer %d: missing planes or BatchNorm affine", l);
  return MOLCLR_OK;
}

struct SegRows {
  int n;
  const int64_t* rows;
  const int64_t* dev;
  int64_t cap;
};
int graph_segments(const molclr_device_graph* g, const int64_t* N, SegRows& out) {
  if (g->segment_nodes_dev) {
    MOLCLR_REQUIRE(g->num_segments >= 1 && g->num_segments <= MOLCLR_MAX_SEGMENTS,
                   "encoder: %d graph segments", g->num_segments);
    out = {g->num_segments, nullptr, g->segment_nodes_dev, *N};
    return MOLCLR_OK;
  }
  if (g->num_segments <= 1) {
    out = {1, N, nullptr, *N};
    return MOLCLR_OK;
  }
  MOLCLR_REQUIRE(g->num_segments <= MOLCLR_MAX_SEGMENTS, "encoder: %d graph segments",
                 g->num_segments);
  int64_t tot = 0;
  for (int s = 0; s < g->num_segments; ++s) tot += g->segment_nodes[s];
  MOLCLR_REQUIRE(tot == *N, "encoder: segment nodes sum to %lld, graph has %lld", (long long)tot,
                 (long long)*N);
  out = {g->num_segments, g->segment_nodes, nullptr, *N};
  return MOLCLR_OK;
}

int seg_bn_fwd(const SegRows& sg, const void* z, const float* gamma, const float* beta,
               float* rmean, float* rvar, int64_t* nbt, void* y, float* mean, float* invstd,
               int64_t D, int dtype, double momentum, double eps, int training, int relu,
               void* ws, size_t ws_bytes, molclr_stream_t stream) {
  if (sg.dev)
    return molclr_batchnorm_seg_fwd_dev(z, gamma, beta, rmean, rvar, nbt, y, mean, invstd, sg.n,
                                        sg.dev, sg.cap, D, dtype, momentum, eps, training, relu,
                                        ws, ws_bytes, stream);
  return molclr_batchnorm_seg_fwd(z, gamma, beta, rmean, rvar, nbt, y, mean, invstd, sg.n,
                                  sg.rows, D, dtype, momentum, eps, training, relu, ws, ws_bytes,
                                  stream);
}
int seg_bn_bwd(const SegRows& sg, const void* dy, const void* z, const float* gamma,
               const float* beta, const float* mean, const float* invstd, void* dz, float* dgamma,
               float* dbeta, int64_t D, int dtype, int relu, int accumulate, float* rowmax,
               float* slot, void* ws, size_t ws_bytes, molclr_stream_t stream) {
  if (sg.dev)
    return molclr_batchnorm_seg_bwd_dev(dy, z, gamma, beta, mean, invstd, dz, dgamma, dbeta, sg.n,
                                        sg.dev, sg.cap, D, dtype, relu, accumulate, rowmax, slot,
                                        ws, ws_bytes, stream);
  if (rowmax)
    return molclr_batchnorm_seg_bwd_max((const float*)dy, (const float*)z, gamma, beta, mean,
                                        invstd, (float*)dz, dgamma, dbeta, sg.n, sg.rows, D, relu,
                                        accumulate, rowmax, slot, ws, ws_bytes, stream);
  return molclr_batchnorm_seg_bwd(dy, z, gamma, beta, mean, invstd, dz, dgamma, dbeta, sg.n,
                                  sg.rows, D, dtype, relu, accumulate, ws, ws_bytes, stream);
}

#define MOLCLR_TRY(expr)      \
  do {                        \
    int rc_ = (expr);         \
    if (rc_) return rc_;      \
  } while (0)

int record_done(void* ev, molclr_stream_t stream) {
  if (ev && hipEventRecord(static_cast<hipEvent_t>(ev), molclr::as_stream(stream)) != hipSuccess) {
    molclr::set_error("encoder_bwd: hipEventRecord failed");
    return MOLCLR_ERR_ARG;
  }
  return MOLCLR_OK;
}

}

MOLCLR_API size_t molclr_gin_encoder_arena_bytes(int L, int64_t N, int64_t D, int dtype) {
  if (L < 1 || L > MOLCLR_MAX_LAYERS) return 0;
  return ArenaLayout(L, N, D, elem_bytes(dtype)).total;
}

constexpr size_t kSlotBytes = MOLCLR_MAX_LAYERS * 2 * kMaxSlotFloats * sizeof(float);
size_t rowmax_first_bytes(int64_t N, int64_t D) {
  const size_t dz = (size_t)molclr_bn_row_parts(D) * N * sizeof(float);
  const size_t agg = molclr_rowmax_bytes(N, D);
  return molclr::align_up(dz > agg ? dz : agg, 256);
}
size_t rowmax_bytes(int64_t N, int64_t D) {
  return molclr::align_up(
      rowmax_first_bytes(N, D) + (size_t)molclr_gemm_row_parts(2 * D) * N * sizeof(float), 256);
}

MOLCLR_API size_t molclr_gin_encoder_workspace_bytes(int L, int64_t N, int64_t D, int dtype) {
  (void)L;
  return molclr::align_up(scratch_bytes(N, D, elem_bytes(dtype)), 256) + kSlotBytes +
         rowmax_bytes(N, D) + kernels_ws(N, D) + 256;
}

MOLCLR_API int molclr_gin_encoder_fwd(const molclr_gin_encoder* e, const int64_t* x,
                                      const molclr_device_graph* g, void* h_out, void* arena,
                                      size_t arena_bytes, void* workspace, size_t workspace_bytes,
                                      molclr_stream_t stream) {
  MOLCLR_TRY(check_encoder(e, g));
  const int L = e->num_layer;
  const int64_t N = g->num_nodes, D = e->dim;
  if (N == 0) return MOLCLR_OK;
  SegRows seg;
  MOLCLR_TRY(graph_segments(g, &g->num_nodes, seg));
  MOLCLR_REQUIRE(x && h_out && arena, "gin_encoder_fwd: null pointer");
  const bool bf = e->dtype == MOLCLR_DTYPE_BF16;
  const size_t es = elem_bytes(e->dtype);
  const ArenaLayout lay(L, N, D, es);
  MOLCLR_REQUIRE_WS(arena_bytes, lay.total);
  MOLCLR_REQUIRE_WS(workspace_bytes, molclr_gin_encoder_workspace_bytes(L, N, D, e->dtype));
  char* A = (char*)arena;
  auto F = [&](size_t off) { return (float*)(A + off); };
  auto H = [&](size_t off) { return (uint16_t*)(A + off); };
  float* ragg = (float*)((char*)workspace + molclr::align_up(scratch_bytes(N, D, es), 256) +
                         kSlotBytes);
  float* ra1 = (float*)((char*)ragg + rowmax_first_bytes(N, D));
  void* kws = (char*)ragg + rowmax_bytes(N, D);
  const size_t kws_bytes = kernels_ws(N, D);
  const bool h3 = !bf && e->fp32_gemm != 0;
  const bool h3f = h3 && (e->fp32_gemm & 2);
  float* fmax = F(lay.smax);

  void* h = A + lay.h0;
  if (bf)
    MOLCLR_TRY(molclr_atom_embed_fwd_bf16(x, e->x_embedding1, e->x_embedding2, (uint16_t*)h, N, D,
                                          e->n_atom, e->n_chiral, e->status, stream));
  else
    MOLCLR_TRY(molclr_atom_embed_fwd(x, e->x_embedding1, e->x_embedding2, (float*)h, N, D,
                                     e->n_atom, e->n_chiral, e->status, stream));
  float* Ec = F(lay.ec);
  const int64_t nz = h3 ? (int64_t)(lay.bmax - lay.smax) / 4 + (int64_t)L * 2 * kMaxSlotFloats : 0;
  MOLCLR_TRY(molclr::edge_tables_combine_zero(L, e->edge_embedding1, e->edge_embedding2, Ec, D,
                                              h3 ? fmax : nullptr, nz, stream));
  for (int l = 0; l < L; ++l) {
    const bool last = l == L - 1;
    void* y = last ? h_out : A + lay.h[l];
    const float* Ecl = Ec + (size_t)l * MOLCLR_NUM_ECOMB * D;
    if (bf) {
      uint16_t *agg = H(lay.agg[l]), *a1 = H(lay.a1[l]), *z = H(lay.z[l]);
      MOLCLR_TRY(molclr_gine_aggregate_fwd_bf16((const uint16_t*)h, g->rowptr, g->col, g->ecode,
                                                g->nbr, Ecl, agg, N, D, stream));
      if (D % 64 == 0)
        MOLCLR_TRY(molclr_gemm_bf16_bits(agg, e->mlp0_planes[l], a1, N, 2 * D, D, D, 2 * D,
                                         MOLCLR_EPI_BIAS_RELU, e->mlp0_bias[l],
                                         (uint32_t*)(A + lay.bits[l]), nullptr, stream));
      else
        MOLCLR_TRY(molclr_gemm_bf16(agg, e->mlp0_planes[l], a1, N, 2 * D, D, D, 2 * D,
                                    MOLCLR_EPI_BIAS_RELU, e->mlp0_bias[l], nullptr, 0, stream));
      MOLCLR_TRY(molclr_gemm_bf16(a1, e->mlp2_planes[l], z, N, D, 2 * D, 2 * D, D,
                                  MOLCLR_EPI_BIAS, e->mlp2_bias[l], nullptr, 0, stream));
      MOLCLR_TRY(seg_bn_fwd(seg, z, e->bn_weight[l], e->bn_bias[l], e->bn_running_mean[l],
                            e->bn_running_var[l], e->bn_num_batches_tracked[l], y, F(lay.mean[l]),
                            F(lay.invstd[l]), D, MOLCLR_DTYPE_BF16, e->momentum, e->eps,
                            e->training, last ? 0 : 1, kws, kws_bytes, stream));
    } else {
      float *agg = F(lay.agg[l]), *a1 = F(lay.a1[l]), *z = F(lay.z[l]);
      float* sl = fmax + 2 * l * kMaxSlotFloats;
      if (h3f)
        MOLCLR_TRY(molclr_gine_aggregate_fwd_rowmax((const float*)h, g->rowptr, g->col, g->ecode,
                                                    g->nbr, Ecl, agg, N, D, ragg, nullptr,
                                                    stream));
      else
        MOLCLR_TRY(molclr_gine_aggregate_fwd((const float*)h, g->rowptr, g->col, g->ecode, g->nbr,
                                             Ecl, agg, N, D, stream));
      if (h3f) {
        const uint16_t* p0 = e->mlp0_planes[l];
        const uint16_t* p2 = e->mlp2_planes[l];
        MOLCLR_TRY(molclr_gemm_f32_h3_bits(agg, ragg, (int)molclr_rowmax_layout(D), p0, a1, N,
                                           2 * D, D, D, 2 * D, MOLCLR_EPI_BIAS_RELU,
                                           e->mlp0_bias[l], nullptr, 0, nullptr,
                                           sl + kMaxSlotFloats, ra1, sl,
                                           (uint32_t*)(A + lay.bits[l]), stream));
        MOLCLR_TRY(molclr_gemm_f32_h3(a1, ra1, (int)molclr_gemm_row_parts(2 * D), p2, z, N, D,
                                      2 * D, 2 * D, D, MOLCLR_EPI_BIAS, e->mlp2_bias[l], nullptr, 0,
                                      nullptr,
                                      nullptr, nullptr, nullptr, stream));
      } else {
        if (h3)
          MOLCLR_TRY(molclr_gemm_f32_bplanes_max(agg, e->mlp0_planes[l], a1, N, 2 * D, D, D, 2 * D,
                                                 MOLCLR_EPI_BIAS_RELU, e->mlp0_bias[l], nullptr, 0,
                                                 fmax + 2 * l * kMaxSlotFloats,
                                                 fmax + (2 * l + 1) * kMaxSlotFloats, nullptr,
                                                 (uint32_t*)(A + lay.bits[l]), kws, kws_bytes,
                                                 stream));
        else
          MOLCLR_TRY(molclr_gemm_f32_bplanes(agg, e->mlp0_planes[l], a1, N, 2 * D, D, D, 2 * D, 0,
                                             MOLCLR_EPI_BIAS_RELU, e->mlp0_bias[l], nullptr, 0, kws,
                                             kws_bytes, stream));
        MOLCLR_TRY(molclr_gemm_f32_bplanes(a1, e->mlp2_planes[l], z, N, D, 2 * D, 2 * D, D, 0,
                                           MOLCLR_EPI_BIAS, e->mlp2_bias[l], nullptr, 0, kws,
                                           kws_bytes, stream));
      }
      MOLCLR_TRY(seg_bn_fwd(seg, z, e->bn_weight[l], e->bn_bias[l], e->bn_running_mean[l],
                            e->bn_running_var[l], e->bn_num_batches_tracked[l], y, F(lay.mean[l]),
                            F(lay.invstd[l]), D, MOLCLR_DTYPE_F32, e->momentum, e->eps,
                            e->training, last ? 0 : 1, kws, kws_bytes, stream));
    }
    h = y;
  }
  return MOLCLR_OK;
}

MOLCLR_API int molclr_gin_encoder_bwd(const molclr_gin_encoder* e,
                                      const molclr_gin_encoder_grads* gr, const int64_t* x,
                                      const molclr_device_graph* g, const void* dh_out,
                                      const void* arena, size_t arena_bytes, void* workspace,
                                      size_t workspace_bytes, molclr_stream_t stream) {
  MOLCLR_TRY(check_encoder(e, g));
  MOLCLR_REQUIRE(gr, "gin_encoder_bwd: null grads");
  MOLCLR_REQUIRE(e->training, "gin_encoder_bwd: backward through eval-mode BatchNorm");
  const int L = e->num_layer;
  const int64_t N = g->num_nodes, D = e->dim;
  if (N == 0) return MOLCLR_OK;
  SegRows seg;
  MOLCLR_TRY(graph_segments(g, &g->num_nodes, seg));
  MOLCLR_REQUIRE(x && dh_out && arena, "gin_encoder_bwd: null pointer");
  const bool bf = e->dtype == MOLCLR_DTYPE_BF16;
  const size_t es = elem_bytes(e->dtype);
  const ArenaLayout lay(L, N, D, es);
  MOLCLR_REQUIRE_WS(arena_bytes, lay.total);
  MOLCLR_REQUIRE_WS(workspace_bytes, molclr_gin_encoder_workspace_bytes(L, N, D, e->dtype));
  const char* A = (const char*)arena;
  auto F = [&](size_t off) { return (const float*)(A + off); };
  char* S = (char*)workspace;
  void* dh = S;
  void* dz = S + (size_t)N * D * es;
  void* dagg = S + 2 * (size_t)N * D * es;
  void* dz1 = S + 3 * (size_t)N * D * es;
  float* bmax = const_cast<float*>(F(lay.bmax));
  float* rdz = (float*)(S + molclr::align_up(scratch_bytes(N, D, es), 256)) +
               kSlotBytes / sizeof(float);
  float* rdz1 = (float*)((char*)rdz + rowmax_first_bytes(N, D));
  void* kws = (char*)rdz + rowmax_bytes(N, D);
  const size_t kws_bytes = kernels_ws(N, D);
  const int dt = bf ? MOLCLR_DTYPE_BF16 : MOLCLR_DTYPE_F32;
  const bool h3 = !bf && e->fp32_gemm != 0;
  const float* fmax = F(lay.smax);

  const void* dy = dh_out;
  for (int l = L - 1; l >= 0; --l) {
    const void* agg = A + lay.agg[l];
    const void* a1 = A + lay.a1[l];
    const void* z = A + lay.z[l];
    const bool last = l == L - 1;
    MOLCLR_REQUIRE(gr->bn_weight[l] && gr->bn_bias[l], "gin_encoder_bwd: BatchNorm grads needed");
    if (h3) {
      MOLCLR_TRY(seg_bn_bwd(seg, dy, z, e->bn_weight[l], e->bn_bias[l], F(lay.mean[l]),
                            F(lay.invstd[l]), dz, gr->bn_weight[l], gr->bn_bias[l], D,
                            MOLCLR_DTYPE_F32, last ? 0 : 1, 1, rdz, nullptr, kws, kws_bytes,
                            stream));
    } else {
      MOLCLR_TRY(seg_bn_bwd(seg, dy, z, e->bn_weight[l], e->bn_bias[l], F(lay.mean[l]),
                            F(lay.invstd[l]), dz, gr->bn_weight[l], gr->bn_bias[l], D, dt,
                            last ? 0 : 1, 1, nullptr, nullptr, kws, kws_bytes, stream));
    }
    if (bf) {
      const uint16_t *hz = (const uint16_t*)dz, *ha1 = (const uint16_t*)a1;
      if (gr->mlp2_weight[l] || gr->mlp2_bias[l]) {
        MOLCLR_REQUIRE(gr->mlp2_weight[l], "gin_encoder_bwd: bf16 needs the weight gradient");
        MOLCLR_TRY(molclr_linear_wgrad_bf16(hz, ha1, gr->mlp2_weight[l], gr->mlp2_bias[l], N, D,
                                            2 * D, D, 2 * D, 1, kws, kws_bytes, stream));
      }
      if (D % 64 == 0)
        MOLCLR_TRY(molclr_gemm_bf16_bits(hz, e->mlp2_planes_t[l], (uint16_t*)dz1, N, 2 * D, D, D,
                                         2 * D, MOLCLR_EPI_RELU_MASK, nullptr, nullptr,
                                         (const uint32_t*)(A + lay.bits[l]), stream));
      else
        MOLCLR_TRY(molclr_gemm_bf16(hz, e->mlp2_planes_t[l], (uint16_t*)dz1, N, 2 * D, D, D, 2 * D,
                                    MOLCLR_EPI_RELU_MASK, nullptr, ha1, 2 * D, stream));
      if (gr->mlp0_weight[l] || gr->mlp0_bias[l]) {
        MOLCLR_REQUIRE(gr->mlp0_weight[l], "gin_encoder_bwd: bf16 needs the weight gradient");
        MOLCLR_TRY(molclr_linear_wgrad_bf16((const uint16_t*)dz1, (const uint16_t*)agg,
                                            gr->mlp0_weight[l], gr->mlp0_bias[l], N, 2 * D, D,
                                            2 * D, D, 1, kws, kws_bytes, stream));
      }
      MOLCLR_TRY(molclr_gemm_bf16((const uint16_t*)dz1, e->mlp0_planes_t[l], (uint16_t*)dagg, N,
                                  D, 2 * D, 2 * D, D, MOLCLR_EPI_NONE, nullptr, nullptr, 0, stream));
      MOLCLR_TRY(molclr_gine_aggregate_bwd_bf16((const uint16_t*)dagg, g->rowptr_t, g->col_t,
                                                g->nbr_t, g->ecount, (uint16_t*)dh,
// ... 272 lines not shown
```

### molclr_amd/csrc/norm.hip

```cpp
#include "common.h"

#include <math.h>

namespace {

constexpr int kT = 256;

__host__ __device__ __forceinline__ int64_t band_parts(int64_t rows, int band) {
  const int64_t unit = (int64_t)band * 16;
  int64_t P = (rows + unit - 1) / unit;
  if (P > 1024) P = 1024;
  if (P < 1) P = 1;
  return P;
}

int64_t band_parts_bound(int64_t rows, int band, int nseg) {
  const int64_t unit = (int64_t)band * 16;
  int64_t P = (rows + unit - 1) / unit + nseg;
  if (P > (int64_t)nseg * 1024) P = (int64_t)nseg * 1024;
  return P;
}

__global__ void k_colsum_partial(const float4* __restrict__ X, int64_t rows, int d4, int64_t ld4,
                                 int band, int64_t rows_per_part, float4* __restrict__ partial) {
  extern __shared__ __attribute__((aligned(16))) float4 red[];
  const int tid = threadIdx.x;
  const bool live = tid < band * d4;
  const int r = live ? tid / d4 : 0, c = live ? tid - r * d4 : 0;
  const int64_t beg = (int64_t)blockIdx.x * rows_per_part;
  int64_t end = beg + rows_per_part;
  if (end > rows) end = rows;
  float4 acc = f4zero();
  if (live) {
#pragma unroll 4
    for (int64_t i = beg + r; i < end; i += band) acc = f4add(acc, X[i * ld4 + c]);
  }
  if (live) red[r * d4 + c] = acc;
  __syncthreads();
  if (live && r == 0) {
    float4 s = red[c];
    for (int q = 1; q < band; ++q) s = f4add(s, red[q * d4 + c]);
    partial[(int64_t)blockIdx.x * d4 + c] = s;
  }
}

constexpr int kRedCols = 4, kRedLanes = 256;

template <typename T>
__device__ __forceinline__ T lane_tree_sum(T (*red)[kRedCols], int rl, int cl, T v) {
  red[rl][cl] = v;
  __syncthreads();
#pragma unroll
  for (int stride = kRedLanes / 2; stride > 0; stride >>= 1) {
    if (rl < stride) red[rl][cl] = v = v + red[rl + stride][cl];
    __syncthreads();
  }
  return v;
}

__device__ __forceinline__ float lane_fold(const float* __restrict__ partial, int64_t P,
                                           int64_t cols, int64_t c, int rl) {
  float a0 = 0.f, a1 = 0.f, a2 = 0.f, a3 = 0.f;
  int64_t p = rl;
  for (; p + 3 * kRedLanes < P; p += 4 * kRedLanes) {
    a0 += partial[p * cols + c];
    a1 += partial[(p + kRedLanes) * cols + c];
    a2 += partial[(p + 2 * kRedLanes) * cols + c];
    a3 += partial[(p + 3 * kRedLanes) * cols + c];
  }
  for (; p < P; p += kRedLanes) a0 += partial[p * cols + c];
  return (a0 + a1) + (a2 + a3);
}

__global__ __launch_bounds__(kRedCols* kRedLanes) void k_colsum_final(
    const float* __restrict__ partial, int64_t P, int64_t cols, float* __restrict__ out,
    int accumulate) {
  __shared__ float red[kRedLanes][kRedCols];
  const int cl = threadIdx.x % kRedCols, rl = threadIdx.x / kRedCols;
  const int64_t c = (int64_t)blockIdx.x * kRedCols + cl;
  const float acc = c < cols ? lane_fold(partial, P, cols, c, rl) : 0.f;
  const float s = lane_tree_sum(red, rl, cl, acc);
  if (rl == 0 && c < cols) out[c] = accumulate ? out[c] + s : s;
}

struct Segs {
  int n;
  int band;
  int64_t rows[MOLCLR_MAX_SEGMENTS];
  const int64_t* drows;
};

__device__ __forceinline__ int64_t seg_n(const Segs& sg, int s) {
  return sg.drows ? sg.drows[s] : sg.rows[s];
}

struct SegAt {
  int s;
  int64_t row0, row1, part0, P, rpp;
};
__device__ __forceinline__ SegAt seg_info(const Segs& sg, int s) {
  int64_t r = 0, p = 0;
  for (int q = 0; q < s; ++q) {
    const int64_t n = seg_n(sg, q);
    r += n;
    p += band_parts(n, sg.band);
  }
  const int64_t n = seg_n(sg, s), P = band_parts(n, sg.band);
  return {s, r, r + n, p, P, (n > 0 ? n + P - 1 : P) / P};
}
__device__ __forceinline__ SegAt seg_of_part(const Segs& sg, int64_t b) {
  int64_t r = 0, p = 0;
  for (int s = 0; s < sg.n; ++s) {
    const int64_t n = seg_n(sg, s), P = band_parts(n, sg.band);
    if (b < p + P) return {s, r, r + n, p, P, (n > 0 ? n + P - 1 : P) / P};
    r += n;
    p += P;
  }
  return {-1, r, r, p, 0, 1};
}
__device__ __forceinline__ int64_t row_of(int64_t t, int d4, int64_t total4) {
  return total4 <= 0x7FFFFFFF ? (int64_t)((uint32_t)t / (uint32_t)d4) : t / d4;
}
__device__ __forceinline__ int seg_of_row(const Segs& sg, int64_t i) {
  int64_t r = 0;
  for (int s = 0; s < sg.n; ++s) {
    r += seg_n(sg, s);
    if (i < r) return s;
  }
  return -1;
}

struct Welford4 {
  float n;
  float4 mean, m2;
};

__device__ __forceinline__ void chan_merge(float& na, float4& ma, float4& qa, float nb, float4 mb,
                                           float4 qb) {
  if (nb == 0.f) return;
  if (na == 0.f) {
    na = nb;
    ma = mb;
    qa = qb;
    return;
  }
  float n = na + nb;
  float wb = nb / n, wab = na * nb / n;
  float4 d = make_float4(mb.x - ma.x, mb.y - ma.y, mb.z - ma.z, mb.w - ma.w);
  ma = make_float4(ma.x + d.x * wb, ma.y + d.y * wb, ma.z + d.z * wb, ma.w + d.w * wb);
  qa = make_float4(qa.x + qb.x + d.x * d.x * wab, qa.y + qb.y + d.y * d.y * wab,
                   qa.z + qb.z + d.z * d.z * wab, qa.w + qb.w + d.w * d.w * wab);
  na = n;
}

template <typename St>
__global__ void k_bn_stats_partial(const typename St::T* __restrict__ z, int d4, int band, Segs sg,
                                   float4* __restrict__ pmean, float4* __restrict__ pm2,
                                   float* __restrict__ pn) {
  extern __shared__ __attribute__((aligned(16))) float4 red[];
  const int tid = threadIdx.x;
  const bool live = tid < band * d4;
  const int r = live ? tid / d4 : 0, c = live ? tid - r * d4 : 0;
  const SegAt at = seg_of_part(sg, blockIdx.x);
  if (at.s < 0) return;
  const int64_t beg = at.row0 + (blockIdx.x - at.part0) * at.rpp;
  int64_t end = beg + at.rpp;
  if (end > at.row1) end = at.row1;
  float n = 0.f;
  float4 mean = f4zero(), m2 = f4zero();
  if (live) {
#pragma unroll 4
    for (int64_t i = beg + r; i < end; i += band) {
      float4 x = St::ld(z, i * d4 + c);
      n += 1.f;
      float inv = 1.f / n;
      float4 d = make_float4(x.x - mean.x, x.y - mean.y, x.z - mean.z, x.w - mean.w);
      mean = make_float4(mean.x + d.x * inv, mean.y + d.y * inv, mean.z + d.z * inv,
                         mean.w + d.w * inv);
      m2 = make_float4(m2.x + d.x * (x.x - mean.x), m2.y + d.y * (x.y - mean.y),
                       m2.z + d.z * (x.z - mean.z), m2.w + d.w * (x.w - mean.w));
    }
    red[r * d4 + c] = mean;
    red[(band + r) * d4 + c] = m2;
  }
  __syncthreads();
  if (live && r == 0) {
    int64_t cnt = end > beg ? end - beg : 0;
    float na = (float)(cnt > 0 ? (cnt + band - 1) / band : 0);
    float4 ma = red[c], qa = red[band * d4 + c];
    for (int q = 1; q < band; ++q) {
      float nb = (float)(cnt > q ? (cnt - q + band - 1) / band : 0);
      chan_merge(na, ma, qa, nb, red[q * d4 + c], red[(band + q) * d4 + c]);
    }
    pmean[(int64_t)blockIdx.x * d4 + c] = ma;
    pm2[(int64_t)blockIdx.x * d4 + c] = qa;
    if (c == 0) pn[blockIdx.x] = (float)cnt;
  }
}

__device__ __forceinline__ void bn_coeffs(float gamma, float beta, float mean, float invstd,
                                          float& scale, float& shift) {
  scale = gamma * invstd;
  shift = __fmaf_rn(-mean, scale, beta);
}

__device__ __forceinline__ void chan1(float& n, float& mean, float& m2, float nb, float mb, float qb) {
  if (nb == 0.f) return;
  if (n == 0.f) {
    n = nb;
    mean = mb;
    m2 = qb;
    return;
// ... 19 lines not shown
  const int half = rl / kSegLanes, sl = rl % kSegLanes;
  const int64_t c = (int64_t)blockIdx.x * kRedCols + cl;
  for (int s0 = 0; s0 < sg.n; s0 += 2) {
    const int s = s0 + half;
    float n = 0.f, mean = 0.f, m2 = 0.f;
    if (s < sg.n && c < D) {
      const SegAt at = seg_info(sg, s);
      const int64_t P = at.P;
      const float* sm = pmean + at.part0 * D;
      const float* sq = pm2 + at.part0 * D;
      const float* sn = pn + at.part0;
      for (int64_t p = sl; p < P; p += 4 * kSegLanes) {
        float bn[4], bm[4], bq[4];
#pragma unroll
        for (int u = 0; u < 4; ++u) {
          const int64_t q = p + u * kSegLanes;
          const bool in = q < P;
          bn[u] = in ? sn[q] : 0.f;
          bm[u] = in ? sm[q * D + c] : 0.f;
          bq[u] = in ? sq[q * D + c] : 0.f;
        }
#pragma unroll
        for (int u = 0; u < 4; ++u) chan1(n, mean, m2, bn[u], bm[u], bq[u]);
      }
    }
    __syncthreads();
    rn[rl][cl] = n;
    rm[rl][cl] = mean;
    rq[rl][cl] = m2;
    __syncthreads();
#pragma unroll
    for (int stride = kSegLanes / 2; stride > 0; stride >>= 1) {
      if (sl < stride) {
        chan1(n, mean, m2, rn[rl + stride][cl], rm[rl + stride][cl], rq[rl + stride][cl]);
        rn[rl][cl] = n;
        rm[rl][cl] = mean;
        rq[rl][cl] = m2;
      }
      __syncthreads();
    }
    if (rl == 0 && c < D) {
      for (int h = 0; h < 2 && s0 + h < sg.n; ++h) {
        const int ss = s0 + h;
        const float nn = rn[h * kSegLanes][cl], mu = rm[h * kSegLanes][cl];
        const float q2 = rq[h * kSegLanes][cl];
        const float var = q2 / nn;
        const float invstd = 1.0f / sqrtf(var + eps);
        save_mean[ss * D + c] = mu;
        save_invstd[ss * D + c] = invstd;
        if (running_mean) running_mean[c] = (1.f - momentum) * running_mean[c] + momentum * mu;
        if (running_var) {
          const float unbiased = nn > 1.f ? q2 / (nn - 1.f) : var;
          running_var[c] = (1.f - momentum) * running_var[c] + momentum * unbiased;
        }
        float sc, sh;
        bn_coeffs(gamma ? gamma[c] : 1.f, beta ? beta[c] : 0.f, mu, invstd, sc, sh);
        scale[ss * D + c] = sc;
        shift[ss * D + c] = sh;
      }
    }
  }
}

__global__ void k_bn_eval_coeffs(const float* __restrict__ gamma, const float* __restrict__ beta,
                                 const float* __restrict__ running_mean,
                                 const float* __restrict__ running_var, int64_t D, int nseg,
                                 float eps, float* __restrict__ save_mean,
                                 float* __restrict__ save_invstd, float* __restrict__ scale,
                                 float* __restrict__ shift) {
  int64_t c = (int64_t)blockIdx.x * blockDim.x + threadIdx.x;
  if (c >= D) return;
  float mean = running_mean[c];
  float invstd = 1.0f / sqrtf(running_var[c] + eps);
  float sc, sh;
  bn_coeffs(gamma ? gamma[c] : 1.f, beta ? beta[c] : 0.f, mean, invstd, sc, sh);
  for (int s = 0; s < nseg; ++s) {
    if (save_mean) save_mean[s * D + c] = mean;
    if (save_invstd) save_invstd[s * D + c] = invstd;
    scale[s * D + c] = sc;
    shift[s * D + c] = sh;
  }
}

__device__ __forceinline__ float bn_apply1(float z, float sc, float sh) { return __fmaf_rn(z, sc, sh); }

template <typename St, int U = 1>
__global__ __launch_bounds__(kT) void k_bn_apply(const typename St::T* __restrict__ z,
                                                 const float4* __restrict__ scale,
                                                 const float4* __restrict__ shift,
                                                 typename St::T* __restrict__ y, int64_t total4,
                                                 int d4, int relu, Segs sg) {
  int64_t t = (int64_t)blockIdx.x * blockDim.x + threadIdx.x;
  if (t >= total4 / U) return;
  const int64_t u0 = t * U;
  const int64_t i = row_of(u0, d4, total4);
  const int c = (int)(u0 - i * d4);
  const int s = seg_of_row(sg, i);
  float4 v[U];
  if (s < 0) {
    if constexpr (U == 2) St::st2(y, t, f4zero(), f4zero());
    else St::st(y, t, f4zero());
    return;
  }
  if constexpr (U == 2) St::ld2(z, t, v[0], v[1]);
  else v[0] = St::ld(z, t);
#pragma unroll
  for (int j = 0; j < U; ++j) {
    const float4 sc = scale[s * d4 + c + j], sh = shift[s * d4 + c + j];
    float4 o = make_float4(bn_apply1(v[j].x, sc.x, sh.x), bn_apply1(v[j].y, sc.y, sh.y),
                           bn_apply1(v[j].z, sc.z, sh.z), bn_apply1(v[j].w, sc.w, sh.w));
    if (relu) o = make_float4(fmaxf(o.x, 0.f), fmaxf(o.y, 0.f), fmaxf(o.z, 0.f), fmaxf(o.w, 0.f));
    v[j] = o;
  }
  if constexpr (U == 2) St::st2(y, t, v[0], v[1]);
  else St::st(y, t, v[0]);
}

__device__ __forceinline__ void bn_coeffs4(const float* gamma, const float* beta, float4 mu,
                                           float4 is, int c, float4& sc, float4& sh) {
  float4 g = gamma ? reinterpret_cast<const float4*>(gamma)[c] : make_float4(1.f, 1.f, 1.f, 1.f);
  float4 b = beta ? reinterpret_cast<const float4*>(beta)[c] : f4zero();
  bn_coeffs(g.x, b.x, mu.x, is.x, sc.x, sh.x);
  bn_coeffs(g.y, b.y, mu.y, is.y, sc.y, sh.y);
  bn_coeffs(g.z, b.z, mu.z, is.z, sc.z, sh.z);
  bn_coeffs(g.w, b.w, mu.w, is.w, sc.w, sh.w);
}

template <typename St>
__global__ void k_bn_bwd_partial(const typename St::T* __restrict__ dy,
                                 const typename St::T* __restrict__ z,
                                 const float4* __restrict__ mean, const float4* __restrict__ invstd,
                                 const float* __restrict__ gamma, const float* __restrict__ beta,
                                 int d4, int band, Segs sg, int relu, float4* __restrict__ p1,
                                 float4* __restrict__ p2) {
  extern __shared__ __attribute__((aligned(16))) float4 red[];
  const int tid = threadIdx.x;
  const bool live = tid < band * d4;
  const int r = live ? tid / d4 : 0, c = live ? tid - r * d4 : 0;
  const SegAt at = seg_of_part(sg, blockIdx.x);
  if (at.s < 0) return;
  const int s = at.s;
  const int64_t beg = at.row0 + (blockIdx.x - at.part0) * at.rpp;
  int64_t end = beg + at.rpp;
  if (end > at.row1) end = at.row1;
  float4 s1 = f4zero(), s2 = f4zero();
  if (live) {
    float4 mu = mean[s * d4 + c], is = invstd[s * d4 + c], sc, sh;
    bn_coeffs4(gamma, beta, mu, is, c, sc, sh);
    constexpr int U = 8;
    for (int64_t i0 = beg + r; i0 < end; i0 += U * (int64_t)band) {
      float4 gv[U], xv[U];
#pragma unroll
      for (int u = 0; u < U; ++u) {
        const int64_t i = i0 + (int64_t)u * band;
        const int64_t ii = i < end ? i : i0;
        gv[u] = St::ld(dy, ii * d4 + c);
        xv[u] = St::ld(z, ii * d4 + c);
      }
#pragma unroll
      for (int u = 0; u < U; ++u) {
        if (i0 + (int64_t)u * band >= end) break;
        float4 g = gv[u];
        const float4 x = xv[u];
        if (relu) {
          g.x = bn_apply1(x.x, sc.x, sh.x) > 0.f ? g.x : 0.f;
          g.y = bn_apply1(x.y, sc.y, sh.y) > 0.f ? g.y : 0.f;
          g.z = bn_apply1(x.z, sc.z, sh.z) > 0.f ? g.z : 0.f;
          g.w = bn_apply1(x.w, sc.w, sh.w) > 0.f ? g.w : 0.f;
// ... 318 lines not shown
    *out = s;
  }
}

}

size_t molclr_colsum_ws(int64_t rows, int64_t cols) {
  molclr::Band b = molclr::make_band(cols);
  return (size_t)band_parts(rows, b.band) * cols * sizeof(float) + 256;
}

int molclr_colsum_impl(const float* X, float* out, int64_t rows, int64_t cols, int64_t ld,
                       int accumulate, molclr::Workspace& w, hipStream_t s) {
  MOLCLR_REQUIRE(cols > 0 && cols % 4 == 0 && ld % 4 == 0, "colsum: cols/ld must be multiples of 4");
  molclr::Band b = molclr::make_band(cols);
  int64_t P = band_parts(rows, b.band);
  float* partial = w.take<float>(P * cols);
  if (!w.ok()) {
    molclr::set_error("colsum: workspace too small");
    return MOLCLR_ERR_WORKSPACE;
  }
  int64_t rpp = molclr::ceil_div(rows > 0 ? rows : 1, P);
  size_t lds = (size_t)b.band * b.d4 * sizeof(float4);
  hipLaunchKernelGGL(k_colsum_partial, dim3(P), dim3(b.threads), lds, s, (const float4*)X, rows,
                     b.d4, ld / 4, b.band, rpp, (float4*)partial);
  hipLaunchKernelGGL(k_colsum_final, dim3(molclr::ceil_div(cols, kRedCols)), dim3(kRedCols * kRedLanes), 0, s, partial, P,
                     cols, out, accumulate);
  MOLCLR_LAUNCHED();
  return MOLCLR_OK;
}

MOLCLR_API size_t molclr_colsum_f32_workspace_bytes(int64_t rows, int64_t cols) {
  return molclr_colsum_ws(rows, cols);
}

MOLCLR_API int molclr_colsum_f32(const float* X, float* out, int64_t rows, int64_t cols,
                                 int64_t ld, int accumulate, void* workspace,
                                 size_t workspace_bytes, molclr_stream_t stream) {
  MOLCLR_REQUIRE_WS(workspace_bytes, molclr_colsum_ws(rows, cols));
  molclr::Workspace w(workspace, workspace_bytes);
  return molclr_colsum_impl(X, out, rows, cols, ld, accumulate, w, molclr::as_stream(stream));
}

namespace {

int make_segs(int nseg, const int64_t* seg_rows, const int64_t* drows, int64_t cap, int64_t D,
              Segs& sg, int64_t& P, int64_t& rows) {
  MOLCLR_REQUIRE(nseg >= 1 && nseg <= MOLCLR_MAX_SEGMENTS && (seg_rows || drows),
                 "batchnorm: %d segments (1..%d)", nseg, MOLCLR_MAX_SEGMENTS);
  const molclr::Band b = molclr::make_band(D);
  sg.n = nseg;
  sg.band = b.band;
  sg.drows = drows;
  P = 0;
  rows = 0;
  for (int s = 0; s < MOLCLR_MAX_SEGMENTS; ++s) sg.rows[s] = 0;
  if (drows) {
    MOLCLR_REQUIRE(cap >= 0, "batchnorm: negative row capacity");
    P = band_parts_bound(cap, b.band, nseg);
    rows = cap;
    return MOLCLR_OK;
  }
  for (int s = 0; s < nseg; ++s) {
    MOLCLR_REQUIRE(seg_rows[s] >= 0, "batchnorm: negative segment rows");
    sg.rows[s] = seg_rows[s];
    P += band_parts(seg_rows[s], b.band);
    rows += seg_rows[s];
  }
  return MOLCLR_OK;
}

size_t bn_ws_bytes(int64_t P, int64_t D, int nseg) {
  molclr::Workspace w(nullptr, 0);
  w.take<float>(P * D);
  w.take<float>(P * D);
  w.take<float>(P);
  w.take<float>(nseg * D);
  w.take<float>(nseg * D);
  w.take<float>(nseg * D);
  w.take<float>(nseg * D);
  return w.used + 256;
}

template <typename St>
int bn_fwd(const void* zv, const float* gamma, const float* beta, float* running_mean,
           float* running_var, int64_t* nbt, void* yv, float* save_mean, float* save_invstd,
           int nseg, const int64_t* seg_rows, int64_t D, double momentum, double eps, int training,
           int relu, void* workspace, size_t workspace_bytes, hipStream_t s,
           const int64_t* drows = nullptr, int64_t cap = 0) {
  Segs sg;
  int64_t P = 0, rows = 0;
  if (int rc = make_segs(nseg, seg_rows, drows, cap, D, sg, P, rows)) return rc;
  MOLCLR_REQUIRE(D > 0 && D % 4 == 0, "batchnorm_fwd: dim must be a multiple of 4");
  for (int q = 0; q < nseg && !drows; ++q)
    MOLCLR_REQUIRE(!training || seg_rows[q] > 1,
                   "batchnorm_fwd: need more than 1 row per segment when training");
  MOLCLR_REQUIRE(training || (running_mean && running_var), "batchnorm_fwd: eval needs running stats");
  MOLCLR_REQUIRE(save_mean && save_invstd && (rows == 0 || zv), "batchnorm_fwd: null pointer");
  MOLCLR_REQUIRE_WS(workspace_bytes, bn_ws_bytes(P, D, nseg));
  const auto* z = static_cast<const typename St::T*>(zv);
  auto* y = static_cast<typename St::T*>(yv);
  const molclr::Band b = molclr::make_band(D);
  molclr::Workspace w(workspace, workspace_bytes);
  float* pmean = w.take<float>(P * D);
  float* pm2 = w.take<float>(P * D);
  float* pn = w.take<float>(P);
  float* scale = w.take<float>(nseg * D);
  float* shift = w.take<float>(nseg * D);
  if (training) {
    const size_t lds = 2 * (size_t)b.band * b.d4 * sizeof(float4);
    hipLaunchKernelGGL(k_bn_stats_partial<St>, dim3((unsigned)P), dim3(b.threads), lds, s, z, b.d4,
                       b.band, sg, (float4*)pmean, (float4*)pm2, pn);
    hipLaunchKernelGGL(k_bn_stats_final, dim3(molclr::ceil_div(D, kRedCols)),
                       dim3(kRedCols * kRedLanes), 0, s, pmean, pm2, pn, sg, D, gamma, beta,
                       running_mean, running_var, save_mean, save_invstd, scale, shift,
                       (float)momentum, (float)eps, nbt);
  } else {
    hipLaunchKernelGGL(k_bn_eval_coeffs, dim3(molclr::ceil_div(D, kT)), dim3(kT), 0, s, gamma,
                       beta, running_mean, running_var, D, nseg, (float)eps, save_mean,
                       save_invstd, scale, shift);
  }
  const int64_t total4 = rows * (D / 4);
  if (total4 > 0 && y) {
    if (St::kBytes == 2 && D % 8 == 0)
      hipLaunchKernelGGL((k_bn_apply<St, 2>), dim3(molclr::ceil_div(total4 / 2, kT)), dim3(kT), 0,
                         s, z, (const float4*)scale, (const float4*)shift, y, total4, (int)(D / 4),
                         relu, sg);
    else
      hipLaunchKernelGGL((k_bn_apply<St, 1>), dim3(molclr::ceil_div(total4, kT)), dim3(kT), 0, s,
                         z, (const float4*)scale, (const float4*)shift, y, total4, (int)(D / 4),
                         relu, sg);
  }
  MOLCLR_LAUNCHED();
  return MOLCLR_OK;
}

int bn_row_parts(int64_t D) { return (int)((D / 4 + 62) / 64) + 1; }

template <typename St>
int bn_bwd(const void* dyv, const void* zv, const float* gamma, const float* beta,
           const float* save_mean, const float* save_invstd, void* dzv, float* dgamma,
           float* dbeta, int nseg, const int64_t* seg_rows, int64_t D, int relu, int accumulate,
           void* workspace, size_t workspace_bytes, hipStream_t s, float* rowparts = nullptr,
           float* slot = nullptr, const int64_t* drows = nullptr, int64_t cap = 0) {
  Segs sg;
  int64_t P = 0, rows = 0;
  if (int rc = make_segs(nseg, seg_rows, drows, cap, D, sg, P, rows)) return rc;
  MOLCLR_REQUIRE(D > 0 && D % 4 == 0, "batchnorm_bwd: dim must be a multiple of 4");
  MOLCLR_REQUIRE(rows > 0 && dyv && zv && save_mean && save_invstd && dzv, "batchnorm_bwd: bad args");
  for (int q = 0; q < nseg && !drows; ++q)
    MOLCLR_REQUIRE(seg_rows[q] > 0, "batchnorm_bwd: empty segment");
  MOLCLR_REQUIRE_WS(workspace_bytes, bn_ws_bytes(P, D, nseg));
  const auto* dy = static_cast<const typename St::T*>(dyv);
  const auto* z = static_cast<const typename St::T*>(zv);
  auto* dz = static_cast<typename St::T*>(dzv);
  const molclr::Band b = molclr::make_band(D);
  molclr::Workspace w(workspace, workspace_bytes);
  float* p1 = w.take<float>(P * D);
  float* p2 = w.take<float>(P * D);
  w.take<float>(P);
  w.take<float>(nseg * D);
  w.take<float>(nseg * D);
  float* k1 = w.take<float>(nseg * D);
  float* k2 = w.take<float>(nseg * D);
  const size_t lds = 2 * (size_t)b.band * b.d4 * sizeof(float4);
  hipLaunchKernelGGL(k_bn_bwd_partial<St>, dim3((unsigned)P), dim3(b.threads), lds, s, dy, z,
                     (const float4*)save_mean, (const float4*)save_invstd, gamma, beta, b.d4,
                     b.band, sg, relu, (float4*)p1, (float4*)p2);
  hipLaunchKernelGGL(k_bn_bwd_final, dim3(molclr::ceil_div(D, kRedCols)), dim3(kRedCols * kRedLanes),
                     0, s, p1, p2, sg, D, dgamma, dbeta, k1, k2, accumulate);
  const int64_t total4 = rows * (D / 4);
  static_assert(kT % 64 == 0, "row parts follow the waves");
  MOLCLR_REQUIRE(!rowparts || rows < (1ll << 31), "batchnorm_seg_bwd_max: too many rows");
  if (St::kBytes == 2 && D % 8 == 0 && !rowparts && !slot)
    hipLaunchKernelGGL(k_bn_bwd_apply2<St>, dim3(molclr::ceil_div(total4 / 2, kT)), dim3(kT), 0, s,
                       dy, z, (const float4*)save_mean, (const float4*)save_invstd, gamma, beta,
                       (const float4*)k1, (const float4*)k2, dz, total4, (int)(D / 4), relu, sg);
  else
    hipLaunchKernelGGL(k_bn_bwd_apply<St>, dim3(molclr::ceil_div(total4, kT)), dim3(kT), 0, s, dy,
                       z, (const float4*)save_mean, (const float4*)save_invstd, gamma, beta,
                       (const float4*)k1, (const float4*)k2, dz, total4, (int)(D / 4), relu, sg,
                       rowparts, bn_row_parts(D), slot);
  MOLCLR_LAUNCHED();
  return MOLCLR_OK;
}

}

size_t molclr_batchnorm_ws_bound(int64_t rows, int64_t D) {
  const molclr::Band b = molclr::make_band(D > 0 ? D : 4);
  return bn_ws_bytes(band_parts_bound(rows, b.band, MOLCLR_MAX_SEGMENTS), D, MOLCLR_MAX_SEGMENTS);
}

MOLCLR_API size_t molclr_batchnorm_seg_workspace_bytes(int nseg, const int64_t* seg_rows,
                                                       int64_t D) {
  Segs sg;
  int64_t P = 0, rows = 0;
  if (make_segs(nseg, seg_rows, nullptr, 0, D > 0 ? D : 4, sg, P, rows)) return 0;
  return bn_ws_bytes(P, D, nseg);
}

MOLCLR_API size_t molclr_batchnorm_workspace_bytes(int64_t rows, int64_t D) {
  return molclr_batchnorm_seg_workspace_bytes(1, &rows, D);
}

MOLCLR_API int molclr_batchnorm_seg_fwd(const void* z, const float* gamma, const float* beta,
                                        float* running_mean, float* running_var,
                                        int64_t* num_batches_tracked, void* y, float* save_mean,
                                        float* save_invstd, int nseg, const int64_t* seg_rows,
                                        int64_t D, int dtype, double momentum, double eps,
                                        int training, int relu, void* workspace,
                                        size_t workspace_bytes, molclr_stream_t stream) {
  hipStream_t s = molclr::as_stream(stream);
  if (dtype == MOLCLR_DTYPE_F32)
    return bn_fwd<StF32>(z, gamma, beta, running_mean, running_var, num_batches_tracked, y,
                         save_mean, save_invstd, nseg, seg_rows, D, momentum, eps, training, relu,
                         workspace, workspace_bytes, s);
  MOLCLR_REQUIRE(dtype == MOLCLR_DTYPE_BF16, "batchnorm_seg_fwd: dtype %d", dtype);
  return bn_fwd<StBF16>(z, gamma, beta, running_mean, running_var, num_batches_tracked, y,
                        save_mean, save_invstd, nseg, seg_rows, D, momentum, eps, training, relu,
                        workspace, workspace_bytes, s);
}

MOLCLR_API int molclr_batchnorm_seg_bwd(const void* dy, const void* z, const float* gamma,
                                        const float* beta, const float* save_mean,
                                        const float* save_invstd, void* dz, float* dgamma,
                                        float* dbeta, int nseg, const int64_t* seg_rows, int64_t D,
                                        int dtype, int relu, int accumulate, void* workspace,
                                        size_t workspace_bytes, molclr_stream_t stream) {
  hipStream_t s = molclr::as_stream(stream);
  if (dtype == MOLCLR_DTYPE_F32)
    return bn_bwd<StF32>(dy, z, gamma, beta, save_mean, save_invstd, dz, dgamma, dbeta, nseg,
                         seg_rows, D, relu, accumulate, workspace, workspace_bytes, s);
  MOLCLR_REQUIRE(dtype == MOLCLR_DTYPE_BF16, "batchnorm_seg_bwd: dtype %d", dtype);
  return bn_bwd<StBF16>(dy, z, gamma, beta, save_mean, save_invstd, dz, dgamma, dbeta, nseg,
                        seg_rows, D, relu, accumulate, workspace, workspace_bytes, s);
}

MOLCLR_API int molclr_bn_row_parts(int64_t dim) { return bn_row_parts(dim); }

MOLCLR_API int molclr_batchnorm_seg_bwd_max(const float* dy, const float* z, const float* gamma,
                                            const float* beta, const float* save_mean,
                                            const float* save_invstd, float* dz, float* dgamma,
                                            float* dbeta, int nseg, const int64_t* seg_rows,
                                            int64_t D, int relu, int accumulate, float* rowmax,
                                            float* slot, void* workspace, size_t workspace_bytes,
                                            molclr_stream_t stream) {
  MOLCLR_REQUIRE(rowmax, "batchnorm_seg_bwd_max: null rowmax");
  return bn_bwd<StF32>(dy, z, gamma, beta, save_mean, save_invstd, dz, dgamma, dbeta, nseg,
                       seg_rows, D, relu, accumulate, workspace, workspace_bytes,
                       molclr::as_stream(stream), rowmax, slot);
}

MOLCLR_API size_t molclr_batchnorm_seg_dev_workspace_bytes(int nseg, int64_t rows_cap, int64_t D) {
  if (nseg < 1 || nseg > MOLCLR_MAX_SEGMENTS) return 0;
  const molclr::Band b = molclr::make_band(D > 0 ? D : 4);
  return bn_ws_bytes(band_parts_bound(rows_cap, b.band, nseg), D, nseg);
}

MOLCLR_API int molclr_batchnorm_seg_fwd_dev(const void* z, const float* gamma, const float* beta,
                                            float* running_mean, float* running_var,
                                            int64_t* num_batches_tracked, void* y, float* save_mean,
                                            float* save_invstd, int nseg,
                                            const int64_t* seg_rows_dev, int64_t rows_cap,
                                            int64_t D, int dtype, double momentum, double eps,
                                            int training, int relu, void* workspace,
                                            size_t workspace_bytes, molclr_stream_t stream) {
  MOLCLR_REQUIRE(seg_rows_dev, "batchnorm_seg_fwd_dev: null seg_rows_dev");
  hipStream_t s = molclr::as_stream(stream);
  if (dtype == MOLCLR_DTYPE_F32)
    return bn_fwd<StF32>(z, gamma, beta, running_mean, running_var, num_batches_tracked, y,
                         save_mean, save_invstd, nseg, nullptr, D, momentum, eps, training, relu,
                         workspace, workspace_bytes, s, seg_rows_dev, rows_cap);
  MOLCLR_REQUIRE(dtype == MOLCLR_DTYPE_BF16, "batchnorm_seg_fwd_dev: dtype %d", dtype);
  return bn_fwd<StBF16>(z, gamma, beta, running_mean, running_var, num_batches_tracked, y,
                        save_mean, save_invstd, nseg, nullptr, D, momentum, eps, training, relu,
                        workspace, workspace_bytes, s, seg_rows_dev, rows_cap);
}

MOLCLR_API int molclr_batchnorm_seg_bwd_dev(const void* dy, const void* z, const float* gamma,
                                            const float* beta, const float* save_mean,
                                            const float* save_invstd, void* dz, float* dgamma,
                                            float* dbeta, int nseg, const int64_t* seg_rows_dev,
                                            int64_t rows_cap, int64_t D, int dtype, int relu,
                                            int accumulate, float* rowmax, float* slot,
                                            void* workspace, size_t workspace_bytes,
                                            molclr_stream_t stream) {
  MOLCLR_REQUIRE(seg_rows_dev, "batchnorm_seg_bwd_dev: null seg_rows_dev");
  MOLCLR_REQUIRE(!rowmax || dtype == MOLCLR_DTYPE_F32, "batchnorm_seg_bwd_dev: row maxima are fp32 only");
  hipStream_t s = molclr::as_stream(stream);
  if (dtype == MOLCLR_DTYPE_F32)
    return bn_bwd<StF32>(dy, z, gamma, beta, save_mean, save_invstd, dz, dgamma, dbeta, nseg,
                         nullptr, D, relu, accumulate, workspace, workspace_bytes, s, rowmax, slot,
                         seg_rows_dev, rows_cap);
  MOLCLR_REQUIRE(dtype == MOLCLR_DTYPE_BF16, "batchnorm_seg_bwd_dev: dtype %d", dtype);
  return bn_bwd<StBF16>(dy, z, gamma, beta, save_mean, save_invstd, dz, dgamma, dbeta, nseg,
                        nullptr, D, relu, accumulate, workspace, workspace_bytes, s, nullptr,
                        nullptr, seg_rows_dev, rows_cap);
}

MOLCLR_API int molclr_batchnorm_fwd(const float* z, const float* gamma, const float* beta,
                                    float* running_mean, float* running_var,
                                    int64_t* num_batches_tracked, float* y,
                                    float* save_mean, float* save_invstd, int64_t rows,
                                    int64_t D, double momentum, double eps, int training,
                                    int relu, void* workspace, size_t workspace_bytes,
                                    molclr_stream_t stream) {
  return molclr_batchnorm_seg_fwd(z, gamma, beta, running_mean, running_var, num_batches_tracked,
                                  y, save_mean, save_invstd, 1, &rows, D, MOLCLR_DTYPE_F32,
                                  momentum, eps, training, relu, workspace, workspace_bytes, stream);
}

MOLCLR_API int molclr_batchnorm_bwd(const float* dy, const float* z, const float* gamma,
                                    const float* beta, const float* save_mean,
                                    const float* save_invstd, float* dz, float* dgamma,
                                    float* dbeta, int64_t rows, int64_t D, int relu,
                                    int accumulate, void* workspace, size_t workspace_bytes,
                                    molclr_stream_t stream) {
  return molclr_batchnorm_seg_bwd(dy, z, gamma, beta, save_mean, save_invstd, dz, dgamma, dbeta,
                                  1, &rows, D, MOLCLR_DTYPE_F32, relu, accumulate, workspace,
                                  workspace_bytes, stream);
}

MOLCLR_API int molclr_segment_pool_fwd(const float* h, const int32_t* graph_ptr, float* out,
                                       int64_t G, int64_t D, int mode, molclr_stream_t stream) {
  MOLCLR_REQUIRE(D > 0 && D % 4 == 0, "segment_pool_fwd: dim must be a multiple of 4");
  if (mode != 0 && mode != 1) {
    molclr::set_error("segment_pool_fwd: mode %d unsupported (0 mean, 1 add)", mode);
    return MOLCLR_ERR_UNSUPPORTED;
  }
  if (G == 0) return MOLCLR_OK;
  int d4 = (int)(D / 4);
  hipLaunchKernelGGL(k_pool_fwd<StF32>, dim3(molclr::ceil_div(G * d4, kT)), dim3(kT), 0,
                     molclr::as_stream(stream), h, graph_ptr, (float4*)out, G, d4, mode);
  MOLCLR_LAUNCHED();
  return MOLCLR_OK;
}

MOLCLR_API int molclr_segment_pool_bwd(const float* dout, const int32_t* graph_ptr, float* dh,
                                       int64_t N, int64_t G, int64_t D, int mode,
                                       molclr_stream_t stream) {
  MOLCLR_REQUIRE(D > 0 && D % 4 == 0, "segment_pool_bwd: dim must be a multiple of 4");
  if (mode != 0 && mode != 1) {
    molclr::set_error("segment_pool_bwd: mode %d unsupported (0 mean, 1 add)", mode);
    return MOLCLR_ERR_UNSUPPORTED;
  }
  hipStream_t s = molclr::as_stream(stream);
  if (N == 0) return MOLCLR_OK;
  int d4 = (int)(D / 4);
  const int64_t work = G * d4 > 0 ? G * d4 : 1;
  hipLaunchKernelGGL(k_pool_bwd<StF32>, dim3(molclr::ceil_div(work, kT)), dim3(kT), 0, s,
                     (const float4*)dout, graph_ptr, dh, G, d4, mode, N);
  MOLCLR_LAUNCHED();
  return MOLCLR_OK;
}

MOLCLR_API int molclr_segment_pool_fwd_bf16(const uint16_t* h, const int32_t* graph_ptr,
                                            float* out, int64_t G, int64_t D, int mode,
                                            molclr_stream_t stream) {
  MOLCLR_REQUIRE(D > 0 && D % 4 == 0, "segment_pool_fwd_bf16: dim must be a multiple of 4");
  MOLCLR_REQUIRE(mode == 0 || mode == 1, "segment_pool_fwd_bf16: mode %d (0 mean, 1 add)", mode);
  if (G == 0) return MOLCLR_OK;
// ... 97 lines not shown
```

Measured before the change: 192,800 molecules/s.

## Fuse BatchNorm apply and ReLU into next layer's GINE aggregation source loads

Result: faster. 197,100 molecules/s, median of 6 (+2.2%).

```diff
diff --git a/include/molclr.h b/include/molclr.h
--- a/include/molclr.h
+++ b/include/molclr.h
@@ -138,6 +138,11 @@
                                      const uint8_t* ecode, const uint32_t* nbr, const float* Ec,
                                      float* out, int64_t N, int64_t D, float* rowparts,
                                      float* slot, molclr_stream_t stream);
+int molclr_gine_aggregate_bn_fwd(const float* z, const float* coeffs, int relu, int nseg,
+                                 const int64_t* seg_rows, const int64_t* seg_rows_dev,
+                                 const int32_t* rowptr, const int32_t* col, const uint8_t* ecode,
+                                 const uint32_t* nbr, const float* Ec, float* out, int64_t N,
+                                 int64_t D, float* rowparts, float* slot, molclr_stream_t stream);
 size_t molclr_gine_aggregate_bwd_workspace_bytes(int64_t num_nodes, int64_t dim);
 int molclr_gine_aggregate_bwd(const float* g, const int32_t* rowptr_t, const int32_t* col_t,
                               const uint32_t* nbr_t, const int32_t* ecount, float* dx, float* dE1, float* dE2,
@@ -291,6 +296,21 @@
                                  int64_t rows_cap, int64_t dim, int dtype, double momentum,
                                  double eps, int training, int relu, void* workspace,
                                  size_t workspace_bytes, molclr_stream_t stream);
+int molclr_batchnorm_seg_coeffs(const void* z, const float* gamma, const float* beta,
+                                float* running_mean, float* running_var,
+                                int64_t* num_batches_tracked, float* save_mean,
+                                float* save_invstd, float* coeffs, int nseg,
+                                const int64_t* seg_rows, int64_t dim, int dtype, double momentum,
+                                double eps, int training, void* workspace, size_t workspace_bytes,
+                                molclr_stream_t stream);
+int molclr_batchnorm_seg_coeffs_dev(const void* z, const float* gamma, const float* beta,
+                                    float* running_mean, float* running_var,
+                                    int64_t* num_batches_tracked, float* save_mean,
+                                    float* save_invstd, float* coeffs, int nseg,
+                                    const int64_t* seg_rows_dev, int64_t rows_cap, int64_t dim,
+                                    int dtype, double momentum, double eps, int training,
+                                    void* workspace, size_t workspace_bytes,
+                                    molclr_stream_t stream);
 int molclr_batchnorm_seg_bwd_dev(const void* dy, const void* z, const float* gamma,
                                  const float* beta, const float* save_mean,
                                  const float* save_invstd, void* dz, float* dgamma, float* dbeta,
@@ -490,6 +510,12 @@
                                    const uint8_t* ecode, const uint32_t* nbr, const float* Ec,
                                    uint16_t* out, int64_t num_nodes, int64_t dim,
                                    molclr_stream_t stream);
+int molclr_gine_aggregate_bn_fwd_bf16(const uint16_t* z, const float* coeffs, int relu, int nseg,
+                                      const int64_t* seg_rows, const int64_t* seg_rows_dev,
+                                      const int32_t* rowptr, const int32_t* col,
+                                      const uint8_t* ecode, const uint32_t* nbr, const float* Ec,
+                                      uint16_t* out, int64_t N, int64_t D,
+                                      molclr_stream_t stream);
 int molclr_gine_aggregate_bwd_bf16(const uint16_t* g, const int32_t* rowptr_t,
                                    const int32_t* col_t, const uint32_t* nbr_t,
                                    const int32_t* ecount, uint16_t* dx, float* dE1, float* dE2,
diff --git a/molclr_amd/_lib.py b/molclr_amd/_lib.py
--- a/molclr_amd/_lib.py
+++ b/molclr_amd/_lib.py
@@ -36,6 +36,15 @@
     "molclr_rowmax_bytes": (c_size_t, [_I64, _I64]),
     "molclr_gine_aggregate_fwd_rowmax": (c_int, [_P, _P, _P, _P, _P, _P, _P, _I64, _I64, _P, _P,
                                                  _P]),
+    "molclr_gine_aggregate_bn_fwd": (c_int, [_P, _P, c_int, c_int, _P, _P, _P, _P, _P, _P, _P, _P,
+                                             _I64, _I64, _P, _P, _P]),
+    "molclr_gine_aggregate_bn_fwd_bf16": (c_int, [_P, _P, c_int, c_int, _P, _P, _P, _P, _P, _P, _P,
+                                                  _P, _I64, _I64, _P]),
+    "molclr_batchnorm_seg_coeffs": (c_int, [_P, _P, _P, _P, _P, _P, _P, _P, _P, c_int, _P, _I64,
+                                            c_int, c_double, c_double, c_int, _P, c_size_t, _P]),
+    "molclr_batchnorm_seg_coeffs_dev": (c_int, [_P, _P, _P, _P, _P, _P, _P, _P, _P, c_int, _P, _I64,
+                                                _I64, c_int, c_double, c_double, c_int, _P,
+                                                c_size_t, _P]),
     "molclr_gine_aggregate_bwd_workspace_bytes": (c_size_t, [_I64, _I64]),
     "molclr_gine_aggregate_bwd": (c_int, [_P, _P, _P, _P, _P, _P, _P, _P, _I64, _I64, c_int, _P,
                                           c_size_t, _P]),
diff --git a/molclr_amd/csrc/aggregate.hip b/molclr_amd/csrc/aggregate.hip
--- a/molclr_amd/csrc/aggregate.hip
+++ b/molclr_amd/csrc/aggregate.hip
@@ -266,13 +266,61 @@
   return f4add(x[(int64_t)nbr_node(w) * d4 + c], Ec[nbr_ecomb(w) * d4 + c]);
 }
 
-template <typename St, bool NT = false>
+struct NoSrcArgs {};
+struct BnSrcArgs {
+  const float4* scale;
+  const float4* shift;
+  int relu;
+  Segs sg;
+};
+
+template <typename St>
+__device__ __forceinline__ float4 bn_src_unit(float4 v, float4 sc, float4 sh, bool relu) {
+  float4 o = make_float4(bn_apply1(v.x, sc.x, sh.x), bn_apply1(v.y, sc.y, sh.y),
+                         bn_apply1(v.z, sc.z, sh.z), bn_apply1(v.w, sc.w, sh.w));
+  if (relu) o = make_float4(fmaxf(o.x, 0.f), fmaxf(o.y, 0.f), fmaxf(o.z, 0.f), fmaxf(o.w, 0.f));
+  if constexpr (St::kBytes == 2) {
+    const uint32_t lo = f32x2_to_bf16x2(o.x, o.y), hi = f32x2_to_bf16x2(o.z, o.w);
+    o = make_float4(bf16_to_f32(lo & 0xFFFFu), bf16_to_f32(lo >> 16), bf16_to_f32(hi & 0xFFFFu),
+                    bf16_to_f32(hi >> 16));
+  }
+  return o;
+}
+
+template <typename St, typename SA>
+struct AggSrc {
+  __device__ __forceinline__ AggSrc(const SA&, int64_t, int, int) {}
+  __device__ __forceinline__ float4 operator()(const typename St::T* __restrict__ x,
+                                               int64_t unit) const {
+    return St::ld(x, unit);
+  }
+};
+template <typename St>
+struct AggSrc<St, BnSrcArgs> {
+  float4 sc, sh;
+  bool relu, pad;
+  __device__ __forceinline__ AggSrc(const BnSrcArgs& a, int64_t i, int c, int d4) {
+    const int s = seg_of_row(a.sg, i);
+    pad = s < 0;
+    relu = a.relu != 0;
+    sc = pad ? f4zero() : a.scale[s * d4 + c];
+    sh = pad ? f4zero() : a.shift[s * d4 + c];
+  }
+  __device__ __forceinline__ float4 operator()(const typename St::T* __restrict__ x,
+                                               int64_t unit) const {
+    if (pad) return f4zero();
+    return bn_src_unit<St>(St::ld(x, unit), sc, sh, relu);
+  }
+};
+
+template <typename St, bool NT = false, typename SA = NoSrcArgs>
 __device__ __forceinline__ float4 gine_agg_elem(
     const typename St::T* __restrict__ x, const int32_t* __restrict__ rowptr,
     const int32_t* __restrict__ col, const uint8_t* __restrict__ ecode,
     const uint4* __restrict__ nbr, const float4* __restrict__ Ec, typename St::T* __restrict__ out,
-    int64_t t, int64_t i, int c, int d4) {
-  auto X = [&](int64_t idx) { return St::ld(x, idx); };
+    int64_t t, int64_t i, int c, int d4, const SA& sa) {
+  const AggSrc<St, SA> src(sa, i, c, d4);
+  auto X = [&](int64_t idx) { return src(x, idx); };
   auto msg = [&](uint32_t w) {
     return f4add(X((int64_t)nbr_node(w) * d4 + c), Ec[nbr_ecomb(w) * d4 + c]);
   };
@@ -304,12 +352,12 @@
   return acc;
 }
 
-template <typename St, bool ROWMAX, bool NT = false>
+template <typename St, bool ROWMAX, bool NT = false, typename SA = NoSrcArgs>
 __global__ __launch_bounds__(kT) void k_gine_agg_fwd(
     const typename St::T* __restrict__ x, const int32_t* __restrict__ rowptr,
     const int32_t* __restrict__ col, const uint8_t* __restrict__ ecode,
     const uint4* __restrict__ nbr, const float4* __restrict__ Ec, typename St::T* __restrict__ out,
-    int64_t N, int d4, float* __restrict__ rowparts, int nparts, float* __restrict__ slot) {
+    int64_t N, int d4, float* __restrict__ rowparts, int nparts, float* __restrict__ slot, SA sa) {
   int64_t t = (int64_t)xcd_remap(blockIdx.x, gridDim.x) * blockDim.x + threadIdx.x;
   int64_t i;
   int c;
@@ -325,7 +373,7 @@
     float m = 0.f;
     int row = -1;
     if (t < N * d4) {
-      const float4 v = gine_agg_elem<St, NT>(x, rowptr, col, ecode, nbr, Ec, out, t, i, c, d4);
+      const float4 v = gine_agg_elem<St, NT>(x, rowptr, col, ecode, nbr, Ec, out, t, i, c, d4, sa);
       m = fmaxf(fmaxf(fabsf(v.x), fabsf(v.y)), fmaxf(fabsf(v.z), fabsf(v.w)));
       row = (int)i;
     }
@@ -337,7 +385,7 @@
     return;
   }
   if (t >= N * d4) return;
-  gine_agg_elem<St, NT>(x, rowptr, col, ecode, nbr, Ec, out, t, i, c, d4);
+  gine_agg_elem<St, NT>(x, rowptr, col, ecode, nbr, Ec, out, t, i, c, d4, sa);
 }
 
 template <typename St = StF32>
@@ -559,20 +607,50 @@
   return {e[0], e[1]};
 }
 
+template <typename SA>
+struct AggSrc8 {
+  __device__ __forceinline__ AggSrc8(const SA&, int64_t, int, int) {}
+  __device__ __forceinline__ F8 operator()(const uint16_t* __restrict__ x, int64_t unit) const {
+    return ld8(x, unit);
+  }
+};
+template <>
+struct AggSrc8<BnSrcArgs> {
+  float4 sc[2], sh[2];
+  bool relu, pad;
+  __device__ __forceinline__ AggSrc8(const BnSrcArgs& a, int64_t i, int c, int d8) {
+    const int s = seg_of_row(a.sg, i);
+    pad = s < 0;
+    relu = a.relu != 0;
+#pragma unroll
+    for (int j = 0; j < 2; ++j) {
+      sc[j] = pad ? f4zero() : a.scale[(s * d8 + c) * 2 + j];
+      sh[j] = pad ? f4zero() : a.shift[(s * d8 + c) * 2 + j];
+    }
+  }
+  __device__ __forceinline__ F8 operator()(const uint16_t* __restrict__ x, int64_t unit) const {
+    if (pad) return {f4zero(), f4zero()};
+    const F8 v = ld8(x, unit);
+    return {bn_src_unit<StBF16>(v.a, sc[0], sh[0], relu), bn_src_unit<StBF16>(v.b, sc[1], sh[1], relu)};
+  }
+};
+
+template <typename SA = NoSrcArgs>
 __global__ __launch_bounds__(kT) void k_gine_agg_fwd_b8(
     const uint16_t* __restrict__ x, const int32_t* __restrict__ rowptr,
     const int32_t* __restrict__ col, const uint8_t* __restrict__ ecode,
     const uint4* __restrict__ nbr, const float4* __restrict__ Ec, uint16_t* __restrict__ out,
-    int64_t N, int d8) {
+    int64_t N, int d8, SA sa) {
   int64_t t = (int64_t)xcd_remap(blockIdx.x, gridDim.x) * blockDim.x + threadIdx.x;
   if (t >= N * d8) return;
   const int64_t i = t / d8;
   const int c = (int)(t - i * d8);
+  const AggSrc8<SA> src(sa, i, c, d8);
   auto msg = [&](uint32_t w) {
-    return f8add(ld8(x, (int64_t)nbr_node(w) * d8 + c), ec8(Ec, nbr_ecomb(w), d8, c));
+    return f8add(src(x, (int64_t)nbr_node(w) * d8 + c), ec8(Ec, nbr_ecomb(w), d8, c));
   };
   const uint4 s = nbr[i];
-  const F8 self = ld8(x, t);
+  const F8 self = src(x, t);
   const F8 es = ec8(Ec, MOLCLR_SELF_LOOP_ECOMB, d8, c);
   const uint32_t deg = nbr_degree(s.x);
   F8 acc = {f4zero(), f4zero()};
@@ -587,7 +665,7 @@
     if (deg > 3) acc = f8add(acc, m3);
   } else {
     for (int32_t k = rowptr[i], e = rowptr[i + 1]; k < e; ++k)
-      acc = f8add(acc, f8add(ld8(x, (int64_t)col[k] * d8 + c), ec8(Ec, MOLCLR_ECOMB(ecode[k]), d8, c)));
+      acc = f8add(acc, f8add(src(x, (int64_t)col[k] * d8 + c), ec8(Ec, MOLCLR_ECOMB(ecode[k]), d8, c)));
   }
   st8(out, t, f8add(acc, f8add(self, es)));
 }
@@ -778,7 +856,7 @@
                                                       : k_gine_agg_fwd<StF32, false, false>,
                        dim3(molclr::ceil_div(N * d4, kT)), dim3(kT), 0, molclr::as_stream(stream),
                        x, rowptr, col, ecode, (const uint4*)nbr, (const float4*)Ec, out, N, d4,
-                       nullptr, 0, nullptr);
+                       nullptr, 0, nullptr, NoSrcArgs{});
   MOLCLR_LAUNCHED();
   return MOLCLR_OK;
 }
@@ -810,7 +888,7 @@
                                                       : k_gine_agg_fwd<StF32, true, false>,
                        dim3(molclr::ceil_div(N * d4, kT)), dim3(kT), 0, molclr::as_stream(stream),
                        x, rowptr, col, ecode, (const uint4*)nbr, (const float4*)Ec, out, N, d4,
-                       rowparts, (int)molclr_rowmax_layout(D), slot);
+                       rowparts, (int)molclr_rowmax_layout(D), slot, NoSrcArgs{});
   MOLCLR_LAUNCHED();
   return MOLCLR_OK;
 }
@@ -946,15 +1024,106 @@
   MOLCLR_REQUIRE(x && rowptr && nbr && Ec && out, "gine_aggregate_fwd_bf16: null pointer");
   if (D % 8 == 0) {
     const int d8 = (int)(D / 8);
-    molclr::launch_timed(molclr::kTimeGineAgg, k_gine_agg_fwd_b8, dim3(molclr::ceil_div(N * d8, kT)),
-                         dim3(kT), 0, molclr::as_stream(stream), x, rowptr, col, ecode,
-                         (const uint4*)nbr, (const float4*)Ec, out, N, d8);
+    molclr::launch_timed(molclr::kTimeGineAgg, k_gine_agg_fwd_b8<NoSrcArgs>,
+                         dim3(molclr::ceil_div(N * d8, kT)), dim3(kT), 0, molclr::as_stream(stream),
+                         x, rowptr, col, ecode, (const uint4*)nbr, (const float4*)Ec, out, N, d8,
+                         NoSrcArgs{});
   } else {
     const int d4 = (int)(D / 4);
     molclr::launch_timed(molclr::kTimeGineAgg, k_gine_agg_fwd<StBF16, false>,
                          dim3(molclr::ceil_div(N * d4, kT)), dim3(kT), 0, molclr::as_stream(stream),
                          x, rowptr, col, ecode, (const uint4*)nbr, (const float4*)Ec, out, N, d4,
-                         nullptr, 0, nullptr);
+                         nullptr, 0, nullptr, NoSrcArgs{});
+  }
+  MOLCLR_LAUNCHED();
+  return MOLCLR_OK;
+}
+
+static int agg_bn_args(const char* who, const float* coeffs, int relu, int nseg,
+                       const int64_t* seg_rows, const int64_t* seg_rows_dev, int64_t N, int64_t D,
+                       BnSrcArgs& a) {
+  MOLCLR_REQUIRE(coeffs && ((uintptr_t)coeffs & 15) == 0, "%s: coeffs null or not 16-byte aligned", who);
+  MOLCLR_REQUIRE(nseg >= 1 && nseg <= MOLCLR_MAX_SEGMENTS && (seg_rows || seg_rows_dev),
+                 "%s: %d segments (1..%d)", who, nseg, MOLCLR_MAX_SEGMENTS);
+  a.scale = reinterpret_cast<const float4*>(coeffs);
+  a.shift = reinterpret_cast<const float4*>(coeffs + (size_t)nseg * D);
+  a.relu = relu;
+  a.sg.n = nseg;
+  a.sg.band = 0;
+  a.sg.drows = seg_rows_dev;
+  int64_t tot = 0;
+  for (int s = 0; s < MOLCLR_MAX_SEGMENTS; ++s) {
+    a.sg.rows[s] = (!seg_rows_dev && s < nseg) ? seg_rows[s] : 0;
+    MOLCLR_REQUIRE(a.sg.rows[s] >= 0, "%s: negative segment rows", who);
+    tot += a.sg.rows[s];
+  }
+  MOLCLR_REQUIRE(seg_rows_dev || tot == N, "%s: segments sum to %lld rows, N = %lld", who,
+                 (long long)tot, (long long)N);
+  return MOLCLR_OK;
+}
+
+MOLCLR_API int molclr_gine_aggregate_bn_fwd(const float* z, const float* coeffs, int relu, int nseg,
+                                            const int64_t* seg_rows, const int64_t* seg_rows_dev,
+                                            const int32_t* rowptr, const int32_t* col,
+                                            const uint8_t* ecode, const uint32_t* nbr,
+                                            const float* Ec, float* out, int64_t N, int64_t D,
+                                            float* rowparts, float* slot, molclr_stream_t stream) {
+  MOLCLR_REQUIRE(D > 0 && D % 4 == 0, "gine_aggregate_bn_fwd: dim %lld must be a multiple of 4",
+                 (long long)D);
+  MOLCLR_REQUIRE(N < (1ll << 31), "gine_aggregate_bn_fwd: too many rows");
+  MOLCLR_REQUIRE(rowparts || !slot, "gine_aggregate_bn_fwd: a slot needs rowparts");
+  if (N == 0) return MOLCLR_OK;
+  MOLCLR_REQUIRE(z && rowptr && nbr && Ec && out, "gine_aggregate_bn_fwd: null pointer");
+  BnSrcArgs a;
+  MOLCLR_TRY_RC(agg_bn_args("gine_aggregate_bn_fwd", coeffs, relu, nseg, seg_rows, seg_rows_dev, N,
+                            D, a));
+  const int d4 = (int)(D / 4);
+  const dim3 grid(molclr::ceil_div(N * d4, kT));
+  hipStream_t s = molclr::as_stream(stream);
+  const uint4* nb = (const uint4*)nbr;
+  const float4* ec = (const float4*)Ec;
+  if (rowparts) {
+    const int np = (int)molclr_rowmax_layout(D);
+    molclr::launch_timed(molclr::kTimeGineAgg,
+                         agg_nt() ? k_gine_agg_fwd<StF32, true, true, BnSrcArgs>
+                                  : k_gine_agg_fwd<StF32, true, false, BnSrcArgs>,
+                         grid, dim3(kT), 0, s, z, rowptr, col, ecode, nb, ec, out, N, d4, rowparts,
+                         np, slot, a);
+  } else {
+    molclr::launch_timed(molclr::kTimeGineAgg,
+                         agg_nt() ? k_gine_agg_fwd<StF32, false, true, BnSrcArgs>
+                                  : k_gine_agg_fwd<StF32, false, false, BnSrcArgs>,
+                         grid, dim3(kT), 0, s, z, rowptr, col, ecode, nb, ec, out, N, d4,
+                         (float*)nullptr, 0, (float*)nullptr, a);
+  }
+  MOLCLR_LAUNCHED();
+  return MOLCLR_OK;
+}
+
+MOLCLR_API int molclr_gine_aggregate_bn_fwd_bf16(const uint16_t* z, const float* coeffs, int relu,
+                                                 int nseg, const int64_t* seg_rows,
+                                                 const int64_t* seg_rows_dev,
+                                                 const int32_t* rowptr, const int32_t* col,
+                                                 const uint8_t* ecode, const uint32_t* nbr,
+                                                 const float* Ec, uint16_t* out, int64_t N,
+                                                 int64_t D, molclr_stream_t stream) {
+  MOLCLR_REQUIRE(D > 0 && D % 4 == 0, "gine_aggregate_bn_fwd_bf16: dim must be a multiple of 4");
+  if (N == 0) return MOLCLR_OK;
+  MOLCLR_REQUIRE(z && rowptr && nbr && Ec && out, "gine_aggregate_bn_fwd_bf16: null pointer");
+  BnSrcArgs a;
+  MOLCLR_TRY_RC(agg_bn_args("gine_aggregate_bn_fwd_bf16", coeffs, relu, nseg, seg_rows,
+                            seg_rows_dev, N, D, a));
+  if (D % 8 == 0) {
+    const int d8 = (int)(D / 8);
+    molclr::launch_timed(molclr::kTimeGineAgg, k_gine_agg_fwd_b8<BnSrcArgs>,
+                         dim3(molclr::ceil_div(N * d8, kT)), dim3(kT), 0, molclr::as_stream(stream),
+                         z, rowptr, col, ecode, (const uint4*)nbr, (const float4*)Ec, out, N, d8, a);
+  } else {
+    const int d4 = (int)(D / 4);
+    molclr::launch_timed(molclr::kTimeGineAgg, k_gine_agg_fwd<StBF16, false, false, BnSrcArgs>,
+                         dim3(molclr::ceil_div(N * d4, kT)), dim3(kT), 0, molclr::as_stream(stream),
+                         z, rowptr, col, ecode, (const uint4*)nbr, (const float4*)Ec, out, N, d4,
+                         (float*)nullptr, 0, (float*)nullptr, a);
   }
   MOLCLR_LAUNCHED();
   return MOLCLR_OK;
diff --git a/molclr_amd/csrc/common.h b/molclr_amd/csrc/common.h
--- a/molclr_amd/csrc/common.h
+++ b/molclr_amd/csrc/common.h
@@ -261,6 +261,27 @@
     p[i] = (uint16_t)(f32x2_to_bf16x2(v, 0.f) & 0xFFFFu);
   }
 };
+
+struct Segs {
+  int n;
+  int band;
+  int64_t rows[MOLCLR_MAX_SEGMENTS];
+  const int64_t* drows;
+};
+
+__device__ __forceinline__ int64_t seg_n(const Segs& sg, int s) {
+  return sg.drows ? sg.drows[s] : sg.rows[s];
+}
+__device__ __forceinline__ int seg_of_row(const Segs& sg, int64_t i) {
+  int64_t r = 0;
+  for (int s = 0; s < sg.n; ++s) {
+    r += seg_n(sg, s);
+    if (i < r) return s;
+  }
+  return -1;
+}
+
+__device__ __forceinline__ float bn_apply1(float z, float sc, float sh) { return __fmaf_rn(z, sc, sh); }
 
 __device__ __forceinline__ float wave_sum(float v) {
 #pragma unroll
diff --git a/molclr_amd/csrc/encoder.hip b/molclr_amd/csrc/encoder.hip
--- a/molclr_amd/csrc/encoder.hip
+++ b/molclr_amd/csrc/encoder.hip
@@ -1,10 +1,21 @@
 #include "common.h"
 
+#include <stdlib.h>
+
 namespace {
+
+bool agg_bn() {
+  static const bool on = [] {
+    const char* e = getenv("MOLCLR_AGG_BN");
+    return !(e != nullptr && e[0] == '0');
+  }();
+  return on;
+}
 
 struct ArenaLayout {
   size_t agg[MOLCLR_MAX_LAYERS], a1[MOLCLR_MAX_LAYERS], z[MOLCLR_MAX_LAYERS],
-      h[MOLCLR_MAX_LAYERS], mean[MOLCLR_MAX_LAYERS], invstd[MOLCLR_MAX_LAYERS];
+      h[MOLCLR_MAX_LAYERS], mean[MOLCLR_MAX_LAYERS], invstd[MOLCLR_MAX_LAYERS],
+      coef[MOLCLR_MAX_LAYERS];
   size_t bits[MOLCLR_MAX_LAYERS];
   size_t h0, ec, smax, bmax, total;
   ArenaLayout(int L, int64_t N, int64_t D, size_t es) {
@@ -18,9 +29,10 @@
       agg[l] = off(N * D * es);
       a1[l] = off(N * 2 * D * es);
       z[l] = off(N * D * es);
-      h[l] = off(N * D * es);
+      h[l] = agg_bn() ? 0 : off(N * D * es);
       mean[l] = off(MOLCLR_MAX_SEGMENTS * D * sizeof(float));
       invstd[l] = off(MOLCLR_MAX_SEGMENTS * D * sizeof(float));
+      coef[l] = off(2 * MOLCLR_MAX_SEGMENTS * D * sizeof(float));
       bits[l] = off((size_t)N * ((2 * D + 31) / 32) * sizeof(uint32_t));
     }
     h0 = off(N * D * es);
@@ -109,6 +121,18 @@
   return molclr_batchnorm_seg_fwd(z, gamma, beta, rmean, rvar, nbt, y, mean, invstd, sg.n,
                                   sg.rows, D, dtype, momentum, eps, training, relu, ws, ws_bytes,
                                   stream);
+}
+int seg_bn_coeffs(const SegRows& sg, const void* z, const float* gamma, const float* beta,
+                  float* rmean, float* rvar, int64_t* nbt, float* mean, float* invstd, float* coef,
+                  int64_t D, int dtype, double momentum, double eps, int training, void* ws,
+                  size_t ws_bytes, molclr_stream_t stream) {
+  if (sg.dev)
+    return molclr_batchnorm_seg_coeffs_dev(z, gamma, beta, rmean, rvar, nbt, mean, invstd, coef,
+                                           sg.n, sg.dev, sg.cap, D, dtype, momentum, eps, training,
+                                           ws, ws_bytes, stream);
+  return molclr_batchnorm_seg_coeffs(z, gamma, beta, rmean, rvar, nbt, mean, invstd, coef, sg.n,
+                                     sg.rows, D, dtype, momentum, eps, training, ws, ws_bytes,
+                                     stream);
 }
 int seg_bn_bwd(const SegRows& sg, const void* dy, const void* z, const float* gamma,
                const float* beta, const float* mean, const float* invstd, void* dz, float* dgamma,
@@ -192,6 +216,7 @@
   const bool h3f = h3 && (e->fp32_gemm & 2);
   float* fmax = F(lay.smax);
 
+  const bool fused = agg_bn();
   void* h = A + lay.h0;
   if (bf)
     MOLCLR_TRY(molclr_atom_embed_fwd_bf16(x, e->x_embedding1, e->x_embedding2, (uint16_t*)h, N, D,
@@ -205,12 +230,21 @@
                                               h3 ? fmax : nullptr, nz, stream));
   for (int l = 0; l < L; ++l) {
     const bool last = l == L - 1;
-    void* y = last ? h_out : A + lay.h[l];
+    const bool bn_src = fused && l > 0;
+    const bool bn_next = fused && !last;
+    void* y = last ? h_out : bn_next ? nullptr : A + lay.h[l];
     const float* Ecl = Ec + (size_t)l * MOLCLR_NUM_ECOMB * D;
+    const void* zp = bn_src ? A + lay.z[l - 1] : nullptr;
+    const float* cp = bn_src ? F(lay.coef[l - 1]) : nullptr;
     if (bf) {
       uint16_t *agg = H(lay.agg[l]), *a1 = H(lay.a1[l]), *z = H(lay.z[l]);
-      MOLCLR_TRY(molclr_gine_aggregate_fwd_bf16((const uint16_t*)h, g->rowptr, g->col, g->ecode,
-                                                g->nbr, Ecl, agg, N, D, stream));
+      if (bn_src)
+        MOLCLR_TRY(molclr_gine_aggregate_bn_fwd_bf16((const uint16_t*)zp, cp, 1, seg.n, seg.rows,
+                                                     seg.dev, g->rowptr, g->col, g->ecode, g->nbr,
+                                                     Ecl, agg, N, D, stream));
+      else
+        MOLCLR_TRY(molclr_gine_aggregate_fwd_bf16((const uint16_t*)h, g->rowptr, g->col, g->ecode,
+                                                  g->nbr, Ecl, agg, N, D, stream));
       if (D % 64 == 0)
         MOLCLR_TRY(molclr_gemm_bf16_bits(agg, e->mlp0_planes[l], a1, N, 2 * D, D, D, 2 * D,
                                          MOLCLR_EPI_BIAS_RELU, e->mlp0_bias[l],
@@ -220,14 +254,25 @@
                                     MOLCLR_EPI_BIAS_RELU, e->mlp0_bias[l], nullptr, 0, stream));
       MOLCLR_TRY(molclr_gemm_bf16(a1, e->mlp2_planes[l], z, N, D, 2 * D, 2 * D, D,
                                   MOLCLR_EPI_BIAS, e->mlp2_bias[l], nullptr, 0, stream));
-      MOLCLR_TRY(seg_bn_fwd(seg, z, e->bn_weight[l], e->bn_bias[l], e->bn_running_mean[l],
-                            e->bn_running_var[l], e->bn_num_batches_tracked[l], y, F(lay.mean[l]),
-                            F(lay.invstd[l]), D, MOLCLR_DTYPE_BF16, e->momentum, e->eps,
-                            e->training, last ? 0 : 1, kws, kws_bytes, stream));
+      if (bn_next)
+        MOLCLR_TRY(seg_bn_coeffs(seg, z, e->bn_weight[l], e->bn_bias[l], e->bn_running_mean[l],
+                                 e->bn_running_var[l], e->bn_num_batches_tracked[l],
+                                 F(lay.mean[l]), F(lay.invstd[l]), F(lay.coef[l]), D,
+                                 MOLCLR_DTYPE_BF16, e->momentum, e->eps, e->training, kws,
+                                 kws_bytes, stream));
+      else
+        MOLCLR_TRY(seg_bn_fwd(seg, z, e->bn_weight[l], e->bn_bias[l], e->bn_running_mean[l],
+                              e->bn_running_var[l], e->bn_num_batches_tracked[l], y,
+                              F(lay.mean[l]), F(lay.invstd[l]), D, MOLCLR_DTYPE_BF16, e->momentum,
+                              e->eps, e->training, last ? 0 : 1, kws, kws_bytes, stream));
     } else {
       float *agg = F(lay.agg[l]), *a1 = F(lay.a1[l]), *z = F(lay.z[l]);
       float* sl = fmax + 2 * l * kMaxSlotFloats;
-      if (h3f)
+      if (bn_src)
+        MOLCLR_TRY(molclr_gine_aggregate_bn_fwd((const float*)zp, cp, 1, seg.n, seg.rows, seg.dev,
+                                                g->rowptr, g->col, g->ecode, g->nbr, Ecl, agg, N,
+                                                D, h3f ? ragg : nullptr, nullptr, stream));
+      else if (h3f)
         MOLCLR_TRY(molclr_gine_aggregate_fwd_rowmax((const float*)h, g->rowptr, g->col, g->ecode,
                                                     g->nbr, Ecl, agg, N, D, ragg, nullptr,
                                                     stream));
@@ -262,10 +307,17 @@
                                            MOLCLR_EPI_BIAS, e->mlp2_bias[l], nullptr, 0, kws,
                                            kws_bytes, stream));
       }
-      MOLCLR_TRY(seg_bn_fwd(seg, z, e->bn_weight[l], e->bn_bias[l], e->bn_running_mean[l],
-                            e->bn_running_var[l], e->bn_num_batches_tracked[l], y, F(lay.mean[l]),
-                            F(lay.invstd[l]), D, MOLCLR_DTYPE_F32, e->momentum, e->eps,
-                            e->training, last ? 0 : 1, kws, kws_bytes, stream));
+      if (bn_next)
+        MOLCLR_TRY(seg_bn_coeffs(seg, z, e->bn_weight[l], e->bn_bias[l], e->bn_running_mean[l],
+                                 e->bn_running_var[l], e->bn_num_batches_tracked[l],
+                                 F(lay.mean[l]), F(lay.invstd[l]), F(lay.coef[l]), D,
+                                 MOLCLR_DTYPE_F32, e->momentum, e->eps, e->training, kws, kws_bytes,
+                                 stream));
+      else
+        MOLCLR_TRY(seg_bn_fwd(seg, z, e->bn_weight[l], e->bn_bias[l], e->bn_running_mean[l],
+                              e->bn_running_var[l], e->bn_num_batches_tracked[l], y,
+                              F(lay.mean[l]), F(lay.invstd[l]), D, MOLCLR_DTYPE_F32, e->momentum,
+                              e->eps, e->training, last ? 0 : 1, kws, kws_bytes, stream));
     }
     h = y;
   }
diff --git a/molclr_amd/csrc/norm.hip b/molclr_amd/csrc/norm.hip
--- a/molclr_amd/csrc/norm.hip
+++ b/molclr_amd/csrc/norm.hip
@@ -83,17 +83,6 @@
   if (rl == 0 && c < cols) out[c] = accumulate ? out[c] + s : s;
 }
 
-struct Segs {
-  int n;
-  int band;
-  int64_t rows[MOLCLR_MAX_SEGMENTS];
-  const int64_t* drows;
-};
-
-__device__ __forceinline__ int64_t seg_n(const Segs& sg, int s) {
-  return sg.drows ? sg.drows[s] : sg.rows[s];
-}
-
 struct SegAt {
   int s;
   int64_t row0, row1, part0, P, rpp;
@@ -120,14 +109,6 @@
 }
 __device__ __forceinline__ int64_t row_of(int64_t t, int d4, int64_t total4) {
   return total4 <= 0x7FFFFFFF ? (int64_t)((uint32_t)t / (uint32_t)d4) : t / d4;
-}
-__device__ __forceinline__ int seg_of_row(const Segs& sg, int64_t i) {
-  int64_t r = 0;
-  for (int s = 0; s < sg.n; ++s) {
-    r += seg_n(sg, s);
-    if (i < r) return s;
-  }
-  return -1;
 }
 
 struct Welford4 {
@@ -313,8 +294,6 @@
   }
 }
 
-__device__ __forceinline__ float bn_apply1(float z, float sc, float sh) { return __fmaf_rn(z, sc, sh); }
-
 template <typename St, int U = 1>
 __global__ __launch_bounds__(kT) void k_bn_apply(const typename St::T* __restrict__ z,
                                                  const float4* __restrict__ scale,
@@ -799,13 +778,18 @@
   return w.used + 256;
 }
 
+struct BnPlan {
+  Segs sg;
+  int64_t rows;
+  const float *scale, *shift;
+};
 template <typename St>
-int bn_fwd(const void* zv, const float* gamma, const float* beta, float* running_mean,
-           float* running_var, int64_t* nbt, void* yv, float* save_mean, float* save_invstd,
-           int nseg, const int64_t* seg_rows, int64_t D, double momentum, double eps, int training,
-           int relu, void* workspace, size_t workspace_bytes, hipStream_t s,
-           const int64_t* drows = nullptr, int64_t cap = 0) {
-  Segs sg;
+int bn_fwd_coeffs(const void* zv, const float* gamma, const float* beta, float* running_mean,
+                  float* running_var, int64_t* nbt, float* save_mean, float* save_invstd,
+                  float* coeffs, int nseg, const int64_t* seg_rows, int64_t D, double momentum,
+                  double eps, int training, void* workspace, size_t workspace_bytes, hipStream_t s,
+                  const int64_t* drows, int64_t cap, BnPlan& plan) {
+  Segs& sg = plan.sg;
   int64_t P = 0, rows = 0;
   if (int rc = make_segs(nseg, seg_rows, drows, cap, D, sg, P, rows)) return rc;
   MOLCLR_REQUIRE(D > 0 && D % 4 == 0, "batchnorm_fwd: dim must be a multiple of 4");
@@ -816,7 +800,6 @@
   MOLCLR_REQUIRE(save_mean && save_invstd && (rows == 0 || zv), "batchnorm_fwd: null pointer");
   MOLCLR_REQUIRE_WS(workspace_bytes, bn_ws_bytes(P, D, nseg));
   const auto* z = static_cast<const typename St::T*>(zv);
-  auto* y = static_cast<typename St::T*>(yv);
   const molclr::Band b = molclr::make_band(D);
   molclr::Workspace w(workspace, workspace_bytes);
   float* pmean = w.take<float>(P * D);
@@ -824,6 +807,10 @@
   float* pn = w.take<float>(P);
   float* scale = w.take<float>(nseg * D);
   float* shift = w.take<float>(nseg * D);
+  if (coeffs) {
+    scale = coeffs;
+    shift = coeffs + (size_t)nseg * D;
+  }
   if (training) {
     const size_t lds = 2 * (size_t)b.band * b.d4 * sizeof(float4);
     hipLaunchKernelGGL(k_bn_stats_partial<St>, dim3((unsigned)P), dim3(b.threads), lds, s, z, b.d4,
@@ -837,7 +824,29 @@
                        beta, running_mean, running_var, D, nseg, (float)eps, save_mean,
                        save_invstd, scale, shift);
   }
-  const int64_t total4 = rows * (D / 4);
+  plan.rows = rows;
+  plan.scale = scale;
+  plan.shift = shift;
+  MOLCLR_LAUNCHED();
+  return MOLCLR_OK;
+}
+
+template <typename St>
+int bn_fwd(const void* zv, const float* gamma, const float* beta, float* running_mean,
+           float* running_var, int64_t* nbt, void* yv, float* save_mean, float* save_invstd,
+           int nseg, const int64_t* seg_rows, int64_t D, double momentum, double eps, int training,
+           int relu, void* workspace, size_t workspace_bytes, hipStream_t s,
+           const int64_t* drows = nullptr, int64_t cap = 0) {
+  BnPlan plan;
+  if (int rc = bn_fwd_coeffs<St>(zv, gamma, beta, running_mean, running_var, nbt, save_mean,
+                                 save_invstd, nullptr, nseg, seg_rows, D, momentum, eps, training,
+                                 workspace, workspace_bytes, s, drows, cap, plan))
+    return rc;
+  const auto* z = static_cast<const typename St::T*>(zv);
+  auto* y = static_cast<typename St::T*>(yv);
+  const Segs& sg = plan.sg;
+  const float *scale = plan.scale, *shift = plan.shift;
+  const int64_t total4 = plan.rows * (D / 4);
   if (total4 > 0 && y) {
     if (St::kBytes == 2 && D % 8 == 0)
       hipLaunchKernelGGL((k_bn_apply<St, 2>), dim3(molclr::ceil_div(total4 / 2, kT)), dim3(kT), 0,
@@ -995,6 +1004,50 @@
                         workspace, workspace_bytes, s, seg_rows_dev, rows_cap);
 }
 
+MOLCLR_API int molclr_batchnorm_seg_coeffs(const void* z, const float* gamma, const float* beta,
+                                           float* running_mean, float* running_var,
+                                           int64_t* num_batches_tracked, float* save_mean,
+                                           float* save_invstd, float* coeffs, int nseg,
+                                           const int64_t* seg_rows, int64_t D, int dtype,
+                                           double momentum, double eps, int training,
+                                           void* workspace, size_t workspace_bytes,
+                                           molclr_stream_t stream) {
+  MOLCLR_REQUIRE(coeffs, "batchnorm_seg_coeffs: null coeffs");
+  hipStream_t s = molclr::as_stream(stream);
+  BnPlan plan;
+  if (dtype == MOLCLR_DTYPE_F32)
+    return bn_fwd_coeffs<StF32>(z, gamma, beta, running_mean, running_var, num_batches_tracked,
+                                save_mean, save_invstd, coeffs, nseg, seg_rows, D, momentum, eps,
+                                training, workspace, workspace_bytes, s, nullptr, 0, plan);
+  MOLCLR_REQUIRE(dtype == MOLCLR_DTYPE_BF16, "batchnorm_seg_coeffs: dtype %d", dtype);
+  return bn_fwd_coeffs<StBF16>(z, gamma, beta, running_mean, running_var, num_batches_tracked,
+                               save_mean, save_invstd, coeffs, nseg, seg_rows, D, momentum, eps,
+                               training, workspace, workspace_bytes, s, nullptr, 0, plan);
+}
+
+MOLCLR_API int molclr_batchnorm_seg_coeffs_dev(const void* z, const float* gamma, const float* beta,
+                                               float* running_mean, float* running_var,
+                                               int64_t* num_batches_tracked, float* save_mean,
+                                               float* save_invstd, float* coeffs, int nseg,
+                                               const int64_t* seg_rows_dev, int64_t rows_cap,
+                                               int64_t D, int dtype, double momentum, double eps,
+                                               int training, void* workspace,
+                                               size_t workspace_bytes, molclr_stream_t stream) {
+  MOLCLR_REQUIRE(coeffs && seg_rows_dev, "batchnorm_seg_coeffs_dev: null coeffs / seg_rows_dev");
+  hipStream_t s = molclr::as_stream(stream);
+  BnPlan plan;
+  if (dtype == MOLCLR_DTYPE_F32)
+    return bn_fwd_coeffs<StF32>(z, gamma, beta, running_mean, running_var, num_batches_tracked,
+                                save_mean, save_invstd, coeffs, nseg, nullptr, D, momentum, eps,
+                                training, workspace, workspace_bytes, s, seg_rows_dev, rows_cap,
+                                plan);
+  MOLCLR_REQUIRE(dtype == MOLCLR_DTYPE_BF16, "batchnorm_seg_coeffs_dev: dtype %d", dtype);
+  return bn_fwd_coeffs<StBF16>(z, gamma, beta, running_mean, running_var, num_batches_tracked,
+                               save_mean, save_invstd, coeffs, nseg, nullptr, D, momentum, eps,
+                               training, workspace, workspace_bytes, s, seg_rows_dev, rows_cap,
+                               plan);
+}
+
 MOLCLR_API int molclr_batchnorm_seg_bwd_dev(const void* dy, const void* z, const float* gamma,
                                             const float* beta, const float* save_mean,
                                             const float* save_invstd, void* dz, float* dgamma,
```
